# yuhogun0908/MISOnet

Measured on AMD Instinct MI355X. Metric: utterances/sec MISO1->MVDR->MISO3, 6-mic 16kHz 4s, higher is better.
Workload: dtype f32w; 1 GPU; BASELINE configs[3]: synthetic 6-mic 16 kHz 4 s, full MISO1x6 -> align -> MVDRx2 -> MISO3x2; batch_per_gpu=16, global_batch=16, frames=1001, freq_bins=129, parallelism=utterance-shard x1

## Files before the change

### include/misonet.h

```cpp
#ifndef MISONET_H_
#define MISONET_H_

#ifdef __cplusplus
extern "C" {
#endif

typedef struct misonet_net misonet_net;
typedef struct misonet_pipeline misonet_pipeline;
typedef void* misonet_stream;

enum {
  MISONET_OK = 0,
  MISONET_EINVAL = -1,
  MISONET_ESTATE = -2,
  MISONET_EHIP = -3,
  MISONET_ENOMEM = -4,
  MISONET_ENAN = -5
};

typedef struct {
  int in_ch;
  int out_ch;
  int en_ch[7];
  int de_ch[7];
  int n_freq;
  int tcn_norm;
} misonet_cfg;

const char* misonet_strerror(int code);
const char* misonet_last_error(void);
int misonet_version(void);

int misonet_net_create(const misonet_cfg* cfg, misonet_net** out);
int misonet_net_destroy(misonet_net* net);
int misonet_net_num_tensors(const misonet_net* net);
const char* misonet_net_tensor_name(const misonet_net* net, int i);
long long misonet_net_tensor_numel(const misonet_net* net, int i);
int misonet_net_set_tensor(misonet_net* net, const char* key, const float* host_data, long long numel);
int misonet_net_commit(misonet_net* net);

int misonet_net_set_precision(misonet_net* net, int mode);
int misonet_net_get_precision(const misonet_net* net);

long long misonet_net_workspace_bytes(const misonet_net* net, int n_samples, int n_frames);

int misonet_net_forward(misonet_net* net, int n_seg, const void* const* seg_dev, const int* seg_ch,
                        int B, int T, void* out_dev, void* ws_dev, long long ws_bytes, misonet_stream stream);
int misonet_net_check(misonet_net* net, const void* ws_dev, misonet_stream stream);

int misonet_net_keep_activations(misonet_net* net, int keep);
int misonet_net_buffer_plan(const misonet_net* net, int n_frames, int max_buffers, long long* offset_bytes,
                            long long* size_bytes, int* first_step, int* last_step);
int misonet_net_conv_plan(const misonet_net* net, int mode, int max_layers, int* kind);
int misonet_net_tap_shape(const misonet_net* net, const char* name, int* C, int* F);
int misonet_net_tap(misonet_net* net, const char* name, const void* ws_dev, int B, int T, float* dst_dev,
                    misonet_stream stream);

long long misonet_mvdr_workspace_bytes(int B, int F, int M);
int misonet_mvdr(const void* src_dev, const void* mix_dev, int B, int F, int M, int T, float epsi,
                 void* out_dev, void* ws_dev, long long ws_bytes, misonet_stream stream);
int misonet_mvdr_debug(const void* ws_dev, int B, int F, int M, void* steer_c128_dev, void* w_c128_dev,
                       misonet_stream stream);

long long misonet_pit_scratch_bytes(int B, int S, int F);
int misonet_pit_select(const void* anchor_dev, const void* cand_dev, int B, int S, int T, int F,
                       int* sel_dev, double* dist_dev, long long dist_bytes, misonet_stream stream);

long long misonet_css_scratch_bytes(int K, int S, int F);
int misonet_css_align(const void* est_dev, int K, int S, int T, int F, int hop_frames, const int* perm0_dev,
                      int* perm_dev, double* dist_dev, long long dist_bytes, misonet_stream stream);
int misonet_css_stitch(const float* y_dev, const int* perm_dev, int K, int S, int W, int hop, int first,
                       long long n_out, short* out_i16_dev, float* out_f32_dev, misonet_stream stream);

long long misonet_score_scratch_bytes(int B, int E, int R, long long n_or_F);
int misonet_score_wave(const void* est_dev, int est_is_i16, long long est_sb, long long est_ss, long long est_st,
                       const float* ref_dev, long long ref_sb, long long ref_ss, long long ref_st, int B, int E, int R,
                       long long n, const int* n_valid_dev, double* stats_dev, void* scratch_dev,
                       long long scratch_bytes, misonet_stream stream);
int misonet_score_spec(const void* est_dev, long long est_sb, long long est_ss, long long est_st, const void* ref_dev,
                       long long ref_sb, long long ref_ss, long long ref_st, int B, int E, int R, int T, int F,
                       double* pair_dev, int* perm_dev, double* upit_dev, void* scratch_dev, long long scratch_bytes,
                       misonet_stream stream);

long long misonet_bss_scratch_bytes(int B, int E, int R, long long n, int Q);
int misonet_bss_corr(const void* est_dev, int est_is_i16, long long est_sb, long long est_ss, long long est_st,
                     const float* ref_dev, long long ref_sb, long long ref_ss, long long ref_st, int B, int E, int R,
                     long long n, const int* n_valid_dev, int Q, double* Rrr_dev, double* Rre_dev, double* Eee_dev,
                     void* scratch_dev, long long scratch_bytes, misonet_stream stream);
int misonet_bss_solve(const double* Rrr_dev, const double* Rre_dev, const double* Eee_dev, int B, int E, int R, int Q,
                      double* T_dev, double* A_dev, int* info_dev, void* scratch_dev, long long scratch_bytes,
                      misonet_stream stream);

int misonet_pipeline_create(misonet_net* miso1, misonet_net* miso3, int num_mic, int num_spk, int ref_ch,
                            float epsi, misonet_pipeline** out);
int misonet_pipeline_destroy(misonet_pipeline* p);
long long misonet_pipeline_workspace_bytes(const misonet_pipeline* p, int B, int T);
int misonet_pipeline_run(misonet_pipeline* p, const void* mix_dev, const void* clean_dev, int B, int T,
                         void* out_dev, void* bf_dev, void* miso1_dev, void* ws_dev, long long ws_bytes,
                         misonet_stream stream);
int misonet_pipeline_check(misonet_pipeline* p, const void* ws_dev, misonet_stream stream);
int misonet_pipeline_run_wav(misonet_pipeline* p, const float* wav_dev, const float* clean_wav_dev, int B,
                             int n_samples, void* out_dev, void* bf_dev, void* miso1_dev, void* ws_dev,
                             long long ws_bytes, misonet_stream stream);

int misonet_stft_frames(int n_samples);
long long misonet_stft_workspace_bytes(int B, int M, int n_samples);
int misonet_frontend_init(void);
int misonet_stft(const float* wav_dev, int B, int n_samples, int M, void* out_dev, void* ws_dev, long long ws_bytes,
                 misonet_stream stream);

int misonet_istft(const void* spec_dev, int N, int T, void* out_i16_dev, float* out_f32_dev, misonet_stream stream);

int misonet_profile_begin(int max_launches);
int misonet_profile_end(double* ms_by_kind , long long* launches_by_kind );

int misonet_event_create(void** ev);
int misonet_event_record(void* ev, misonet_stream stream);
int misonet_event_elapsed_ms(void* start, void* stop, float* ms);
int misonet_event_destroy(void* ev);

#ifdef __cplusplus
}
#endif
#endif
```

### misonet_amd/_lib.py

```python
from __future__ import annotations

import ctypes as C
import os

_HERE = os.path.dirname(os.path.abspath(__file__))
LIB_PATH = os.environ.get("MISONET_LIB_PATH") or os.path.join(_HERE, "libmisonet_hip.so")

OK, EINVAL, ESTATE, EHIP, ENOMEM, ENAN = 0, -1, -2, -3, -4, -5


class MisonetError(RuntimeError):
    def __init__(self, code, detail):
        super().__init__(f"libmisonet_hip error {code}: {detail}")
        self.code = code


class Cfg(C.Structure):
    _fields_ = [("in_ch", C.c_int), ("out_ch", C.c_int), ("en_ch", C.c_int * 7), ("de_ch", C.c_int * 7),
                ("n_freq", C.c_int), ("tcn_norm", C.c_int)]


SIGNATURES = {
    "misonet_strerror": (C.c_char_p, [C.c_int]),
    "misonet_last_error": (C.c_char_p, []),
    "misonet_version": (C.c_int, []),
    "misonet_net_create": (C.c_int, [C.POINTER(Cfg), C.POINTER(C.c_void_p)]),
    "misonet_net_destroy": (C.c_int, [C.c_void_p]),
    "misonet_net_num_tensors": (C.c_int, [C.c_void_p]),
    "misonet_net_tensor_name": (C.c_char_p, [C.c_void_p, C.c_int]),
    "misonet_net_tensor_numel": (C.c_longlong, [C.c_void_p, C.c_int]),
    "misonet_net_set_tensor": (C.c_int, [C.c_void_p, C.c_char_p, C.c_void_p, C.c_longlong]),
    "misonet_net_commit": (C.c_int, [C.c_void_p]),
    "misonet_net_set_precision": (C.c_int, [C.c_void_p, C.c_int]),
    "misonet_net_get_precision": (C.c_int, [C.c_void_p]),
    "misonet_net_keep_activations": (C.c_int, [C.c_void_p, C.c_int]),
    "misonet_net_buffer_plan": (C.c_int, [C.c_void_p, C.c_int, C.c_int, C.POINTER(C.c_longlong), C.POINTER(C.c_longlong),
                                          C.POINTER(C.c_int), C.POINTER(C.c_int)]),
    "misonet_net_conv_plan": (C.c_int, [C.c_void_p, C.c_int, C.c_int, C.POINTER(C.c_int)]),
    "misonet_net_workspace_bytes": (C.c_longlong, [C.c_void_p, C.c_int, C.c_int]),
    "misonet_net_forward": (C.c_int, [C.c_void_p, C.c_int, C.POINTER(C.c_void_p), C.POINTER(C.c_int), C.c_int, C.c_int,
                                      C.c_void_p, C.c_void_p, C.c_longlong, C.c_void_p]),
    "misonet_net_check": (C.c_int, [C.c_void_p, C.c_void_p, C.c_void_p]),
    "misonet_net_tap_shape": (C.c_int, [C.c_void_p, C.c_char_p, C.POINTER(C.c_int), C.POINTER(C.c_int)]),
    "misonet_net_tap": (C.c_int, [C.c_void_p, C.c_char_p, C.c_void_p, C.c_int, C.c_int, C.c_void_p, C.c_void_p]),
    "misonet_mvdr_workspace_bytes": (C.c_longlong, [C.c_int, C.c_int, C.c_int]),
    "misonet_mvdr": (C.c_int, [C.c_void_p, C.c_void_p, C.c_int, C.c_int, C.c_int, C.c_int, C.c_float, C.c_void_p,
                               C.c_void_p, C.c_longlong, C.c_void_p]),
    "misonet_mvdr_debug": (C.c_int, [C.c_void_p, C.c_int, C.c_int, C.c_int, C.c_void_p, C.c_void_p, C.c_void_p]),
    "misonet_pit_scratch_bytes": (C.c_longlong, [C.c_int, C.c_int, C.c_int]),
    "misonet_pit_select": (C.c_int, [C.c_void_p, C.c_void_p, C.c_int, C.c_int, C.c_int, C.c_int, C.c_void_p, C.c_void_p,
                                     C.c_longlong, C.c_void_p]),
    "misonet_css_scratch_bytes": (C.c_longlong, [C.c_int, C.c_int, C.c_int]),
    "misonet_css_align": (C.c_int, [C.c_void_p, C.c_int, C.c_int, C.c_int, C.c_int, C.c_int, C.c_void_p, C.c_void_p,
                                    C.c_void_p, C.c_longlong, C.c_void_p]),
    "misonet_css_stitch": (C.c_int, [C.c_void_p, C.c_void_p, C.c_int, C.c_int, C.c_int, C.c_int, C.c_int, C.c_longlong,
                                     C.c_void_p, C.c_void_p, C.c_void_p]),
    "misonet_score_scratch_bytes": (C.c_longlong, [C.c_int, C.c_int, C.c_int, C.c_longlong]),
    "misonet_score_wave": (C.c_int, [C.c_void_p, C.c_int, C.c_longlong, C.c_longlong, C.c_longlong, C.c_void_p, C.c_longlong,
                                     C.c_longlong, C.c_longlong, C.c_int, C.c_int, C.c_int, C.c_longlong, C.c_void_p,
                                     C.c_void_p, C.c_void_p, C.c_longlong, C.c_void_p]),
    "misonet_score_spec": (C.c_int, [C.c_void_p, C.c_longlong, C.c_longlong, C.c_longlong, C.c_void_p, C.c_longlong,
                                     C.c_longlong, C.c_longlong, C.c_int, C.c_int, C.c_int, C.c_int, C.c_int, C.c_void_p,
                                     C.c_void_p, C.c_void_p, C.c_void_p, C.c_longlong, C.c_void_p]),
    "misonet_bss_scratch_bytes": (C.c_longlong, [C.c_int, C.c_int, C.c_int, C.c_longlong, C.c_int]),
    "misonet_bss_corr": (C.c_int, [C.c_void_p, C.c_int, C.c_longlong, C.c_longlong, C.c_longlong, C.c_void_p, C.c_longlong,
                                   C.c_longlong, C.c_longlong, C.c_int, C.c_int, C.c_int, C.c_longlong, C.c_void_p, C.c_int,
                                   C.c_void_p, C.c_void_p, C.c_void_p, C.c_void_p, C.c_longlong, C.c_void_p]),
    "misonet_bss_solve": (C.c_int, [C.c_void_p, C.c_void_p, C.c_void_p, C.c_int, C.c_int, C.c_int, C.c_int, C.c_void_p,
                                    C.c_void_p, C.c_void_p, C.c_void_p, C.c_longlong, C.c_void_p]),
    "misonet_pipeline_create": (C.c_int, [C.c_void_p, C.c_void_p, C.c_int, C.c_int, C.c_int, C.c_float,
                                          C.POINTER(C.c_void_p)]),
    "misonet_pipeline_destroy": (C.c_int, [C.c_void_p]),
    "misonet_pipeline_workspace_bytes": (C.c_longlong, [C.c_void_p, C.c_int, C.c_int]),
    "misonet_pipeline_run": (C.c_int, [C.c_void_p, C.c_void_p, C.c_void_p, C.c_int, C.c_int, C.c_void_p, C.c_void_p,
                                       C.c_void_p, C.c_void_p, C.c_longlong, C.c_void_p]),
    "misonet_pipeline_run_wav": (C.c_int, [C.c_void_p, C.c_void_p, C.c_void_p, C.c_int, C.c_int, C.c_void_p, C.c_void_p,
                                           C.c_void_p, C.c_void_p, C.c_longlong, C.c_void_p]),
    "misonet_stft_frames": (C.c_int, [C.c_int]),
    "misonet_stft_workspace_bytes": (C.c_longlong, [C.c_int, C.c_int, C.c_int]),
    "misonet_stft": (C.c_int, [C.c_void_p, C.c_int, C.c_int, C.c_int, C.c_void_p, C.c_void_p, C.c_longlong, C.c_void_p]),
    "misonet_frontend_init": (C.c_int, []),
    "misonet_istft": (C.c_int, [C.c_void_p, C.c_int, C.c_int, C.c_void_p, C.c_void_p, C.c_void_p]),
    "misonet_pipeline_check": (C.c_int, [C.c_void_p, C.c_void_p, C.c_void_p]),
    "misonet_profile_begin": (C.c_int, [C.c_int]),
    "misonet_profile_end": (C.c_int, [C.POINTER(C.c_double), C.POINTER(C.c_longlong)]),
    "misonet_event_create": (C.c_int, [C.POINTER(C.c_void_p)]),
    "misonet_event_record": (C.c_int, [C.c_void_p, C.c_void_p]),
    "misonet_event_elapsed_ms": (C.c_int, [C.c_void_p, C.c_void_p, C.POINTER(C.c_float)]),
    "misonet_event_destroy": (C.c_int, [C.c_void_p]),
}

_lib = None


def lib():
    global _lib
    if _lib is None:
        if not os.path.exists(LIB_PATH):
            raise ImportError(f"{LIB_PATH} is missing: build the HIP extension first (make -C misonet_amd/csrc). "
                              "misonet_amd has no CPU fallback.")
        import torch
        L = C.CDLL(LIB_PATH)
        for name, (res, args) in SIGNATURES.items():
            fn = getattr(L, name)
            fn.restype = res
            fn.argtypes = args
        _lib = L
    return _lib


def check(code):
    if code != OK:
        L = lib()
        detail = L.misonet_last_error().decode() or L.misonet_strerror(code).decode()
        if code == ENAN:
            raise FloatingPointError(f"libmisonet_hip: {detail}")
        raise MisonetError(code, detail)


def stream_ptr(device=None):
    import torch
    return C.c_void_p(torch.cuda.current_stream(device).cuda_stream)
```

### misonet_amd/csrc/conv.hip

```cpp
#include "conv_select.hpp"
#include <stdlib.h>
#include "conv_epilogue.hpp"

#include <atomic>
#include <type_traits>

namespace mn {

typedef float f32x16 __attribute__((ext_vector_type(16)));
typedef float f32x4 __attribute__((ext_vector_type(4)));
typedef unsigned int u32x4v __attribute__((ext_vector_type(4)));

int conv_cop(int Cout) { return Cout <= 32 ? 32 : 64; }
int conv_rows(int sf, int tr2) { return tr2 ? 3 : sf * (FT - 1) + 3; }
static int f32_rows(const ConvArgs& a) { return a.tr2 ? 5 : a.sf * (FT - 1) + 3; }

template <int NCO, int NR, int SF, bool TR2, int KFMASK, int NCP = CK / 2, bool ROW0 = false>
__device__ __forceinline__ void chunk_mfma(f32x16 (&acc)[NCO][4], const float* s_in, const float* s_w, int frel,
                                           int half, int l31) {
  constexpr int COP = NCO * 32;
  constexpr int NKF = ((KFMASK >> 0) & 1) + ((KFMASK >> 1) & 1) + ((KFMASK >> 2) & 1);
  constexpr int NSTEP = 3 * NKF * NCP;
  const float* wbase = s_w + half * COP + l31;
  const float* ibase[3];
#pragma unroll
  for (int kf = 0; kf < 3; ++kf) {
    const int rl = ROW0 ? 0 : (TR2 ? ((frel + kf) >> 1) : (SF * frel + kf));
    ibase[kf] = s_in + (half * NR + rl) * TW + l31 + 3;
  }
  float av[2][NCO], bv[2][4];
#define MN_LOAD(ST, BUF)                                                                        \
  {                                                                                             \
    constexpr int tap_ = (ST) / NCP, cp_ = (ST) % NCP;                                          \
    constexpr int kt_ = tap_ / NKF, ks_ = tap_ % NKF;                                           \
    constexpr int kf_ = (NKF == 3) ? ks_ : (NKF == 1 ? (KFMASK == 1 ? 0 : (KFMASK == 2 ? 1 : 2)) : (ks_ == 0 ? 0 : 2)); \
    _Pragma("unroll") for (int j = 0; j < NCO; ++j)                                             \
        av[BUF][j] = wbase[((kt_ * 3 + kf_) * CK + cp_ * 2) * COP + j * 32];                    \
    _Pragma("unroll") for (int q = 0; q < 4; ++q)                                               \
        bv[BUF][q] = ibase[kf_][cp_ * 2 * NR * TW + q * 32 + kt_];                              \
  }
  MN_LOAD(0, 0)
#pragma unroll
  for (int st = 0; st < NSTEP; ++st) {
    const int cur = st & 1;
    if (st + 1 < NSTEP) {
      const int nx = st + 1;
      const int tap_ = nx / NCP, cp_ = nx % NCP;
      const int kt_ = tap_ / NKF, ks_ = tap_ % NKF;
      const int kf_ = (NKF == 3) ? ks_ : (NKF == 1 ? (KFMASK == 1 ? 0 : (KFMASK == 2 ? 1 : 2)) : (ks_ == 0 ? 0 : 2));
#pragma unroll
      for (int j = 0; j < NCO; ++j) av[cur ^ 1][j] = wbase[((kt_ * 3 + kf_) * CK + cp_ * 2) * COP + j * 32];
#pragma unroll
      for (int q = 0; q < 4; ++q) bv[cur ^ 1][q] = ibase[kf_][cp_ * 2 * NR * TW + q * 32 + kt_];
    }
    __builtin_amdgcn_sched_barrier(0);
#pragma unroll
    for (int q = 0; q < 4; ++q)
#pragma unroll
      for (int j = 0; j < NCO; ++j)
        acc[j][q] = __builtin_amdgcn_mfma_f32_32x32x2f32(av[cur][j], bv[cur][q], acc[j][q], 0, 0, 0);
    __builtin_amdgcn_sched_barrier(0);
  }
#undef MN_LOAD
}

struct W1dRaw { float d[4]; };
__device__ __forceinline__ W1dRaw w1d_raw(const float* p) { W1dRaw r; r.d[0] = p[0]; r.d[1] = p[1]; r.d[2] = p[2]; r.d[3] = p[3]; return r; }
__device__ __forceinline__ void w1d_vr(const W1dRaw& r, float (&v)[4]) {
  v[0] = r.d[0] - r.d[2]; v[1] = r.d[1] + r.d[2]; v[2] = r.d[2] - r.d[1]; v[3] = r.d[1] - r.d[3];
}
template <int NR, int SF = 2, int NCP = CK / 2, int CP0 = 0, int NKF = 3>
__device__ __forceinline__ void chunk_w1d_s2(f32x16 (&acc)[4][2], const float* s_in, const float* s_w, int frel, int half, int l31) {
  const float* wb = s_w + half * 32 + l31;
  const float* ib0 = s_in + (half * NR + SF * frel) * TW + 2 * l31 + 3;
  constexpr int NSTEP = NKF * NCP;
  W1dRaw r0[2], r1[2];
  float u[2][4];
#define W1D_LOAD(ST, BUF)                                                                        \
  {                                                                                              \
    constexpr int kf_ = (ST) / NCP, cp_ = CP0 + (ST) % NCP;                                      \
    const float* ib_ = ib0 + kf_ * TW + cp_ * 2 * NR * TW;                                       \
    r0[BUF] = w1d_raw(ib_); r1[BUF] = w1d_raw(ib_ + 64);                                         \
    _Pragma("unroll") for (int nu = 0; nu < 4; ++nu) u[BUF][nu] = wb[((nu * 3 + kf_) * CK + cp_ * 2) * 32]; \
  }
  W1D_LOAD(0, 0)
#pragma unroll
  for (int st = 0; st < NSTEP; ++st) {
    const int cur = st & 1;
    if (st + 1 < NSTEP) {
      const int kf_ = (st + 1) / NCP, cp_ = CP0 + (st + 1) % NCP;
      const float* ib_ = ib0 + kf_ * TW + cp_ * 2 * NR * TW;
      r0[cur ^ 1] = w1d_raw(ib_); r1[cur ^ 1] = w1d_raw(ib_ + 64);
#pragma unroll
      for (int nu = 0; nu < 4; ++nu) u[cur ^ 1][nu] = wb[((nu * 3 + kf_) * CK + cp_ * 2) * 32];
    }
    __builtin_amdgcn_sched_barrier(0);
    float v0[4], v1[4];
    w1d_vr(r0[cur], v0);
    w1d_vr(r1[cur], v1);
#pragma unroll
    for (int nu = 0; nu < 4; ++nu) {
      acc[nu][0] = __builtin_amdgcn_mfma_f32_32x32x2f32(u[cur][nu], v0[nu], acc[nu][0], 0, 0, 0);
      acc[nu][1] = __builtin_amdgcn_mfma_f32_32x32x2f32(u[cur][nu], v1[nu], acc[nu][1], 0, 0, 0);
    }
    __builtin_amdgcn_sched_barrier(0);
  }
#undef W1D_LOAD
}
__device__ __forceinline__ void chunk_w1d_tr2(f32x16 (&acc)[4][2], const float* s_in, const float* s_w, int pr, int q, int half, int l31) {
  constexpr int NR = 3;
  const float* wb = s_w + half * 32 + l31;
  const float* ib = s_in + (half * NR + pr) * TW + 2 * l31 + 3 + 64 * q;
  W1dRaw ra[2], rb[2];
  float u0[2][4], u1[2][4], u2[2][4];
#define W1D_LOAD(CP, BUF)                                                                        \
  {                                                                                              \
    ra[BUF] = w1d_raw(ib + (CP) * 2 * NR * TW); rb[BUF] = w1d_raw(ib + (CP) * 2 * NR * TW + TW); \
    _Pragma("unroll") for (int nu = 0; nu < 4; ++nu) {                                           \
      u0[BUF][nu] = wb[((nu * 3 + 0) * CK + (CP) * 2) * 32];                                     \
      u1[BUF][nu] = wb[((nu * 3 + 1) * CK + (CP) * 2) * 32];                                     \
      u2[BUF][nu] = wb[((nu * 3 + 2) * CK + (CP) * 2) * 32];                                     \
    }                                                                                            \
  }
  W1D_LOAD(0, 0)
#pragma unroll
  for (int cp = 0; cp < CK / 2; ++cp) {
    const int cur = cp & 1;
    if (cp + 1 < CK / 2) W1D_LOAD(cp + 1, cur ^ 1)
    __builtin_amdgcn_sched_barrier(0);
    float va[4], vb[4];
    w1d_vr(ra[cur], va);
    w1d_vr(rb[cur], vb);
#pragma unroll
    for (int nu = 0; nu < 4; ++nu) {
      acc[nu][0] = __builtin_amdgcn_mfma_f32_32x32x2f32(u0[cur][nu], va[nu], acc[nu][0], 0, 0, 0);
      acc[nu][1] = __builtin_amdgcn_mfma_f32_32x32x2f32(u1[cur][nu], vb[nu], acc[nu][1], 0, 0, 0);
      acc[nu][0] = __builtin_amdgcn_mfma_f32_32x32x2f32(u2[cur][nu], vb[nu], acc[nu][0], 0, 0, 0);
    }
    __builtin_amdgcn_sched_barrier(0);
  }
#undef W1D_LOAD
}
template <int Q0, int NQ, bool ACT = true>
__device__ __forceinline__ void w1d_epilogue(const ConvArgs& a, f32x16 (&acc)[4][2], int n, int cg, int f, int tq, bool row_ok, int lane,
                                             float* s_red, const float2* s_bc) {
  const int half = lane >> 5, l31 = lane & 31;
  const int T = a.T, Tp = a.Tp;
  const int cbase = cg * 32;
  const unsigned P4 = (unsigned)a.Fout * (unsigned)Tp * 4u;
  const float* ob = a.out + (long long)n * a.out_bstride + (long long)a.out_c0 * a.Fout * Tp;
  const __amdgpu_buffer_rsrc_t rs = make_rsrc_e(reinterpret_cast<unsigned long long>(ob), (unsigned)a.Cout * P4);
  const bool all_t = row_ok && (tq + 64 * NQ <= T);
  float2 bc[16];
#pragma unroll
  for (int r = 0; r < 16; ++r) bc[r] = s_bc[(r & 3) + 8 * (r >> 2) + 4 * half];
  unsigned voff[NQ];
  bool ok[NQ], ok2[NQ];
#pragma unroll
  for (int q = 0; q < NQ; ++q) {
    const int te = tq + 64 * q + 2 * l31;
    ok[q] = row_ok && te < T;
    ok2[q] = ok[q] && te + 1 < T;
    voff[q] = ok[q] ? (unsigned)(f * Tp + te) * 4u + (unsigned)(4 * half) * P4 : 0x80000000u;
  }
  float s1[16], s2[16];
  auto body = [&](auto masked) {
    constexpr bool MASKED = decltype(masked)::value;
#pragma unroll
    for (int r = 0; r < 16; ++r) {
      const int kr = (r & 3) + 8 * (r >> 2);
      const unsigned coff = (unsigned)(cbase + kr) * P4;
      const float b = bc[r].x;
      const f32x2_t cr = {bc[r].y, bc[r].y};
      float a1 = 0.f, a2 = 0.f;
#pragma unroll
      for (int q = 0; q < NQ; ++q) {
        const float m0 = acc[0][Q0 + q][r], m1 = acc[1][Q0 + q][r], m2 = acc[2][Q0 + q][r], m3 = acc[3][Q0 + q][r];
        f32x2_t y = {(m0 + m1) + m2 + b, (m1 - m2) - m3 + b};
        if (ACT) y = elu_fast2(y) - cr;
        typedef unsigned int uu2 __attribute__((ext_vector_type(2)));
        __builtin_amdgcn_raw_buffer_store_b64(__builtin_bit_cast(uu2, y), rs, voff[q] + coff, 0, 0);
        if (!ACT) continue;
        const float ze = (!MASKED || ok[q]) ? y.x : 0.f, zo = (!MASKED || ok2[q]) ? y.y : 0.f;
        a1 += ze + zo;
        a2 = fmaf(ze, ze, fmaf(zo, zo, a2));
      }
      s1[r] = a1;
      s2[r] = a2;
    }
  };
  if (all_t || !ACT) body(std::false_type{}); else body(std::true_type{});
  if (!ACT) return;
  const float x1 = reduce16_halfwave(s1, lane);
  const float x2 = reduce16_halfwave(s2, lane);
  if ((lane & 16) == 0) {
    const int qq = lane & 15;
    const int co_l = (qq & 3) + 8 * (qq >> 2) + 4 * half;
    s_red[co_l * 2 + 0] = x1;
    s_red[co_l * 2 + 1] = x2;
  }
}

template <int NCO, int MODE, int OCTP = 0, bool HALFK = false, bool W1D = false>
__global__ __launch_bounds__(256, ((NCO == 1 && MODE != 2 && OCTP == 0 && !HALFK && !W1D) ? 3 : 2)) void conv3x3_mfma(const ConvArgs a) {
  static_assert(MODE != 2 || NCO == 1, "stride-2 transposed: two output rows per wave, 32-channel groups");
  static_assert(MODE != 4 || W1D, "MODE 4 exists in the W1D form only");
  static_assert(!W1D || (NCO == 1 && OCTP == 0 && (MODE == 0 || (!HALFK && (MODE == 1 || MODE == 2 || MODE == 3 || MODE == 4)))),
                "W1D: the frequency-strided layers and the first layer, 32-channel groups, planar output");
  constexpr int COP = NCO * 32;
  constexpr int NR = MODE == 0 ? 6 : (MODE == 1 ? 9 : (MODE == 2 ? (W1D ? 3 : 5) : (MODE == 4 ? 3 : 1)));
  constexpr int SF = (MODE == 1 || MODE == 4) ? 2 : 1;
  constexpr int NG = MODE == 4 ? 4 : 1;
  constexpr bool TR2 = MODE == 2;
  constexpr int FTO = (TR2 && !W1D) ? 2 * FT : FT;
  constexpr int NTAP = W1D ? 12 : 9;
  constexpr int NW4 = NTAP * CK * COP * NG / 4;
  constexpr int NWI = (NW4 + 255) / 256;
  extern __shared__ __align__(16) float smem[];
  float* s_in = smem;
  float* s_w = s_in + CK * NR * TW;
  float2* s_nrm = reinterpret_cast<float2*>(s_w + NTAP * CK * COP * NG);

  const int tid = threadIdx.x;
  const int lane = tid & 63;
  const int wave = __builtin_amdgcn_readfirstlane(tid >> 6);
  const ConvTile ct = conv_tile(a);
  if (!ct.valid) return;
  const int t0 = ct.t_tile * TT;
  const int f0 = ct.f_tile * FTO;
  const int n = ct.n;
  const int cg = ct.cg;
  const int T = a.T, Tp = a.Tp, Fin = a.Fin, Cin = a.Cin;
  const int nchunk = (Cin + CK - 1) / CK;
  const int fin0 = MODE == 3 ? 0 : (TR2 ? (f0 >> 1) - 1 : SF * f0 - a.padf);

  const float* in_n = a.in + (long long)n * a.in_bstride + (long long)a.in_c0 * Fin * Tp;
  const f32x4* w_g = reinterpret_cast<const f32x4*>((W1D ? a.w1d : a.w) + (long long)cg * NG * nchunk * (NTAP * CK * COP));

  const int sq = tid & 31, sci = tid >> 5;
  const int tg = t0 + 4 * sq;
  const int hr = tid >> 4, hci = (tid >> 1) & 7, hside = tid & 1;
  const int htg = hside ? t0 + TT : t0 - 1;
  const bool hok = (hr < NR) && htg >= 0 && htg < T && (fin0 + hr) >= 0 && (fin0 + hr) < Fin;

  f32x4 pin[NR];
  float ph = 0.f;
  f32x4 pw[NWI];

  const unsigned row_e = (unsigned)Tp;
  const unsigned plane_e = (unsigned)Fin * row_e;
  const unsigned long long pa = reinterpret_cast<unsigned long long>(in_n);
  const unsigned plo = __builtin_amdgcn_readfirstlane((unsigned)pa);
  const unsigned phi = __builtin_amdgcn_readfirstlane((unsigned)(pa >> 32));
  const __amdgpu_buffer_rsrc_t rs_in = __builtin_amdgcn_make_buffer_rsrc(
      reinterpret_cast<void*>(((unsigned long long)phi << 32) | plo), 0,
      __builtin_amdgcn_readfirstlane((int)((unsigned)Cin * plane_e * 4u)), 0x00020000);
  const unsigned tg_e = (unsigned)(tg < Tp ? tg : Tp - 4);
  const bool full_t = (t0 + TT <= T);
  unsigned hoff_b;
  {
    int fh = fin0 + (hr < NR ? hr : NR - 1);
    fh = fh < 0 ? 0 : (fh >= Fin ? Fin - 1 : fh);
    const int th = htg < 0 ? 0 : (htg >= Tp ? Tp - 1 : htg);
    hoff_b = ((unsigned)fh * row_e + (unsigned)th) * 4u;
  }
  unsigned roff_b[NR];
#pragma unroll
  for (int r = 0; r < NR; ++r) {
    int fin = fin0 + r;
    fin = fin < 0 ? 0 : (fin >= Fin ? Fin - 1 : fin);
    roff_b[r] = ((unsigned)fin * row_e + tg_e) * 4u;
  }

#define STAGE_ISSUE_S(KC, PIN, PH, PW)                                                                          \
  {                                                                                              \
    int c_ = (KC) * CK + sci;                                                                    \
    c_ = c_ < Cin ? c_ : Cin - 1;                                                                \
    const unsigned cb_ = (unsigned)c_ * plane_e * 4u;                                            \
    _Pragma("unroll") for (int r = 0; r < NR; ++r) PIN[r] = __builtin_bit_cast(                  \
        f32x4, __builtin_amdgcn_raw_buffer_load_b128(rs_in, cb_ + roff_b[r], 0, 0));             \
    int c2_ = (KC) * CK + hci;                                                                   \
    c2_ = c2_ < Cin ? c2_ : Cin - 1;                                                             \
    PH = __builtin_bit_cast(float, __builtin_amdgcn_raw_buffer_load_b32(                         \
        rs_in, (unsigned)c2_ * plane_e * 4u + hoff_b, 0, 0));                                    \
    const f32x4* wsrc_ = w_g + (unsigned)(KC) * (unsigned)NW4;                                   \
    _Pragma("unroll") for (int i = 0; i < NWI; ++i) {                                            \
      unsigned idx_ = tid + 256 * i;                                                             \
      if (NW4 % 256 != 0) idx_ = idx_ < (unsigned)NW4 ? idx_ : (unsigned)(NW4 - 1);              \
      if (NG > 1) {  \
        constexpr int per_ = NTAP * CK * COP / 4;                                                \
        PW[i] = w_g[(unsigned)((i / (per_ / 256)) * nchunk + (KC)) * (unsigned)per_ + tid + 256 * (i % (per_ / 256))]; \
      } else PW[i] = wsrc_[idx_];                                                                \
    }                                                                                            \
  }

#define STAGE_COMMIT_S(KC, PIN, PH, PW)                                                                         \
  {                                                                                              \
    const float2 m_ = s_nrm[(KC) * CK + sci];                                                    \
    _Pragma("unroll") for (int r = 0; r < NR; ++r) {                                             \
      const int fin_ = fin0 + r;                                                                 \
      f32x4 v_ = {0.f, 0.f, 0.f, 0.f};                                                           \
      if (fin_ >= 0 && fin_ < Fin) {                                                \
        v_.x = fmaf(PIN[r].x, m_.x, m_.y);                                                       \
        v_.y = fmaf(PIN[r].y, m_.x, m_.y);                                                       \
        v_.z = fmaf(PIN[r].z, m_.x, m_.y);                                                       \
        v_.w = fmaf(PIN[r].w, m_.x, m_.y);                                                       \
        if (!full_t) {                                                                           \
          v_.x = (tg + 0 < T) ? v_.x : 0.f;                                                      \
          v_.y = (tg + 1 < T) ? v_.y : 0.f;                                                      \
          v_.z = (tg + 2 < T) ? v_.z : 0.f;                                                      \
          v_.w = (tg + 3 < T) ? v_.w : 0.f;                                                      \
        }                                                                                        \
      }                                                                                          \
      *reinterpret_cast<f32x4*>(s_in + (sci * NR + r) * TW + 4 + 4 * sq) = v_;                   \
    }                                                                                            \
    if (hr < NR) {                                                                               \
      const float2 m2_ = s_nrm[(KC) * CK + hci];                                                 \
      s_in[(hci * NR + hr) * TW + (hside ? TT + 4 : 3)] = hok ? fmaf(PH, m2_.x, m2_.y) : 0.f;    \
    }                                                                                            \
    _Pragma("unroll") for (int i = 0; i < NWI; ++i) {                                            \
      const int idx_ = tid + 256 * i;                                                            \
      if (NW4 % 256 == 0 || idx_ < NW4) reinterpret_cast<f32x4*>(s_w)[idx_] = PW[i];             \
    }                                                                                            \
  }
#define STAGE_ISSUE(KC) STAGE_ISSUE_S(KC, pin, ph, pw)
#define STAGE_COMMIT(KC) STAGE_COMMIT_S(KC, pin, ph, pw)

  const int f = TR2 ? (W1D ? f0 + 2 * (wave >> 1) : f0 + 2 * wave) : (MODE == 4 ? f0 : f0 + wave);
  const bool row_ok = f < a.Fout;
  int nseg = (T - t0 + 31) >> 5;
  nseg = nseg > 4 ? 4 : nseg;

  f32x16 wacc[4][2];
  if (W1D) {
#pragma unroll
    for (int nu = 0; nu < 4; ++nu)
#pragma unroll
      for (int q = 0; q < 2; ++q)
#pragma unroll
        for (int r = 0; r < 16; ++r) wacc[nu][q][r] = 0.f;
  }
  f32x16 acc[NCO][4];
  f32x16 acc_o[NCO][4];
#pragma unroll
  for (int j = 0; j < NCO; ++j)
#pragma unroll
    for (int s = 0; s < 4; ++s)
#pragma unroll
      for (int r = 0; r < 16; ++r) { acc[j][s][r] = 0.f; if (TR2) acc_o[j][s][r] = 0.f; }

  const int half = lane >> 5, l31 = lane & 31;

  STAGE_ISSUE(0)
  float bias_v = 0.f;
  if (W1D && tid < 32 * NG) bias_v = __builtin_nontemporal_load(a.bias + cg * (32 * NG) + tid);
  for (int c = tid; c < nchunk * CK; c += 256) {
    float mean = 0.f, rstd = (c < Cin) ? 1.f : 0.f;
    if (c >= a.ident_c && c < Cin) {
      const dstat_t* st = a.in_stats + ((long long)n * a.in_sstride + a.in_c0 + c) * (2 * DS_NL);
      const double cnt = (double)Fin * (double)T;
      const double m = dstat_read(st) / cnt;
      double var = dstat_read(st + DS_NL) / cnt - m * m;
      var = var > 0.0 ? var : 0.0;
      mean = (float)m;
      rstd = (float)(1.0 / sqrt(var + (double)IN_EPS));
    }
    s_nrm[c] = make_float2(rstd, -mean * rstd);
  }
  float2* s_bc = s_nrm + nchunk * CK;
  if (W1D && tid < 32 * NG) s_bc[tid] = make_float2(bias_v, elu_fast(bias_v));

  __syncthreads();
  STAGE_COMMIT(0)
  __syncthreads();

  for (int kc = 0; kc < nchunk; ++kc) {
    const bool more = (kc + 1 < nchunk);
    if (more) STAGE_ISSUE(kc + 1)
    if (W1D) {
      if (row_ok) {
        if (TR2) chunk_w1d_tr2(wacc, s_in, s_w, wave >> 1, wave & 1, half, l31);
        else if (MODE == 4) chunk_w1d_s2<NR, SF>(wacc, s_in, s_w + wave * (NTAP * CK * COP), 0, half, l31);
        else if (MODE == 3) chunk_w1d_s2<NR, SF, CK / 2, 0, 1>(wacc, s_in, s_w + (2 - wave) * (CK * COP), 0, half, l31);
        else if (HALFK) {
          chunk_w1d_s2<NR, SF, CK / 4, 0>(wacc, s_in, s_w, f - f0, half, l31);
          if (kc != nchunk - 1) chunk_w1d_s2<NR, SF, CK / 4, CK / 4>(wacc, s_in, s_w, f - f0, half, l31);
        } else chunk_w1d_s2<NR, SF>(wacc, s_in, s_w, f - f0, half, l31);
      }
    } else if (row_ok) {
      if (TR2) {
        chunk_mfma<NCO, NR, SF, TR2, 5>(acc, s_in, s_w, f - f0, half, l31);
        chunk_mfma<NCO, NR, SF, TR2, 2>(acc_o, s_in, s_w, f - f0 + 1, half, l31);
      } else if (MODE == 3) {
        chunk_mfma<NCO, NR, SF, TR2, 1, CK / 2, true>(acc, s_in, s_w + (2 - wave) * (CK * COP), 0, half, l31);
      } else if (HALFK && kc == nchunk - 1) {
        chunk_mfma<NCO, NR, SF, TR2, 7, CK / 4>(acc, s_in, s_w, f - f0, half, l31);
      } else {
        chunk_mfma<NCO, NR, SF, TR2, 7>(acc, s_in, s_w, f - f0, half, l31);
      }
    }
    __syncthreads();
    if (more) {
      STAGE_COMMIT(kc + 1)
      __syncthreads();
    }
  }

  float* s_red = smem;
  if (W1D) {
    if (TR2) {
      const int q = wave & 1, rt = 2 * (wave >> 1);
      w1d_epilogue<0, 1>(a, wacc, n, cg, f, t0 + 64 * q, row_ok, lane, s_red + ((rt * 2 + q) * 32) * 2, s_bc);
      w1d_epilogue<1, 1>(a, wacc, n, cg, f + 1, t0 + 64 * q, f + 1 < a.Fout, lane, s_red + (((rt + 1) * 2 + q) * 32) * 2, s_bc);
    } else if (MODE == 4) {
      w1d_epilogue<0, 2>(a, wacc, n, cg * NG + wave, f, t0, row_ok, lane, s_red + wave * (32 * 2), s_bc + wave * 32);
    } else {
      if (MODE == 0 && !a.act) w1d_epilogue<0, 2, false>(a, wacc, n, cg, f, t0, row_ok, lane, s_red + wave * (32 * 2), s_bc);
      else w1d_epilogue<0, 2>(a, wacc, n, cg, f, t0, row_ok, lane, s_red + wave * (32 * 2), s_bc);
    }
    if (a.act) {
      __syncthreads();
      if (MODE == 4) {
        const int g = tid >> 6, co_l = (tid & 63) >> 1, which = tid & 1;
        const int co = (cg * NG + g) * 32 + co_l;
        if (co < a.Cout) {
          float tot = 0.f;
          if (f0 < a.Fout) tot += s_red[(g * 32 + co_l) * 2 + which];
          dstat_add(a.out_stats + (((long long)n * a.out_sstride + a.out_c0 + co) * 2 + which) * DS_NL, (double)tot);
        }
      } else if (tid < 64) {
        const int co_l = tid >> 1, which = tid & 1;
        const int co = cg * 32 + co_l;
        if (co < a.Cout) {
          float tot = 0.f;
          if (TR2) {
            for (int sl = 0; sl < 8; ++sl)
              if (f0 + (sl >> 1) < a.Fout) tot += s_red[(sl * 32 + co_l) * 2 + which];
          } else {
            for (int w = 0; w < FT; ++w)
              if (f0 + w < a.Fout) tot += s_red[(w * 32 + co_l) * 2 + which];
          }
          dstat_add(a.out_stats + (((long long)n * a.out_sstride + a.out_c0 + co) * 2 + which) * DS_NL, (double)tot);
        }
      }
    }
    return;
  }
  if (TR2) {
    conv_epilogue<NCO, 4, OCTP, true>(a, acc, n, cg, f, t0, row_ok, lane, s_red + (2 * wave) * (COP * 2));
    conv_epilogue<NCO, 4, OCTP, true>(a, acc_o, n, cg, f + 1, t0, f + 1 < a.Fout, lane, s_red + (2 * wave + 1) * (COP * 2));
  } else {
    conv_epilogue<NCO, 4, OCTP, true>(a, acc, n, cg, f, t0, row_ok, lane, s_red + wave * (COP * 2));
  }
  if (a.act) {
    __syncthreads();
    if (tid < COP * 2) {
      const int co_l = tid >> 1, which = tid & 1;
      const int co = cg * COP + co_l;
      if (co < a.Cout) {
        float tot = 0.f;
        for (int w = 0; w < FTO; ++w)
          if (f0 + w < a.Fout) tot += s_red[(w * COP + co_l) * 2 + which];
        dstat_add(a.out_stats + (((long long)n * a.out_sstride + a.out_c0 + co) * 2 + which) * DS_NL, (double)tot);
      }
    }
  }
}

#undef STAGE_ISSUE
#undef STAGE_COMMIT
#undef STAGE_ISSUE_S
#undef STAGE_COMMIT_S

static size_t conv_lds_bytes(int NR, int cop, int Cin, int ntap = 9) {
  const int nchunk = (Cin + CK - 1) / CK;
  return (size_t)(CK * NR * TW + ntap * CK * cop) * sizeof(float) + (size_t)(nchunk * CK + 128) * sizeof(float2);
}

template <int NCO, int MODE, int OCTP = 0, bool HALFK = false, bool W1D = false>
static hipError_t set_lds_attr() {
  return hipFuncSetAttribute(reinterpret_cast<const void*>(&conv3x3_mfma<NCO, MODE, OCTP, HALFK, W1D>),
                             hipFuncAttributeMaxDynamicSharedMemorySize, 96 * 1024);
}

hipError_t conv_init() {
  hipError_t e;
  if ((e = set_lds_attr<1, 0>()) != hipSuccess) return e;
  if ((e = set_lds_attr<1, 1>()) != hipSuccess) return e;
  if ((e = set_lds_attr<1, 2>()) != hipSuccess) return e;
  if ((e = set_lds_attr<2, 0>()) != hipSuccess) return e;
  if ((e = set_lds_attr<2, 1>()) != hipSuccess) return e;
  if ((e = set_lds_attr<1, 1, 0, false, true>()) != hipSuccess) return e;
  if ((e = set_lds_attr<1, 2, 0, false, true>()) != hipSuccess) return e;
  if ((e = set_lds_attr<1, 0, 0, true, true>()) != hipSuccess) return e;
  if ((e = set_lds_attr<1, 0, 0, false, true>()) != hipSuccess) return e;
  if ((e = set_lds_attr<1, 4, 0, false, true>()) != hipSuccess) return e;
  if ((e = set_lds_attr<1, 3, 0, false, true>()) != hipSuccess) return e;
  if ((e = set_lds_attr<1, 3>()) != hipSuccess) return e;
  if ((e = set_lds_attr<2, 3>()) != hipSuccess) return e;
  if ((e = set_lds_attr<1, 0, 3>()) != hipSuccess) return e;
  if ((e = set_lds_attr<1, 2, 3>()) != hipSuccess) return e;
  if ((e = set_lds_attr<2, 0, 3>()) != hipSuccess) return e;
#ifdef MISONET_EXPERIMENTS
  if ((e = set_lds_attr<1, 0, 4>()) != hipSuccess) return e;
  if ((e = set_lds_attr<1, 2, 4>()) != hipSuccess) return e;
  if ((e = set_lds_attr<2, 0, 4>()) != hipSuccess) return e;
  if ((e = set_lds_attr<1, 0, 4, true>()) != hipSuccess) return e;
#endif
  if ((e = set_lds_attr<1, 0, 0, true>()) != hipSuccess) return e;
  return set_lds_attr<1, 0, 3, true>();
}

int device_cus() {
  static std::atomic<int> cus[64];
  int dev = 0;
  if (hipGetDevice(&dev) != hipSuccess || dev < 0 || dev >= 64) return -1;
  int c = cus[dev].load(std::memory_order_relaxed);
  if (!c) {
    if (hipDeviceGetAttribute(&c, hipDeviceAttributeMultiprocessorCount, dev) != hipSuccess || c <= 0) return -1;
    cus[dev].store(c, std::memory_order_relaxed);
  }
  return c;
}

int conv_xcd_env() {
  static int v = -1;
  if (v < 0) v = exp_env("MISONET_XCD", 1);
  return v;
}

template <class S> static int conv_mode(const S& a) { return a.tr2 ? 2 : (a.sf == 2 ? 1 : ((a.padf == 2 && a.Fin == 1 && !a.out_oct) ? 3 : 0)); }
static bool w1d_row(const ConvShape& s) { return !s.tr2 && s.act && s.Fout == 1 && s.Fin == 3 && s.padf == 0 && s.Cout % 128 == 0; }

bool conv_w1d_ok(const ConvShape& s) {
  if (s.in_oct || s.out_oct) return false;
  if (conv_mode(s) != 0) return s.act;
  return !s.transposed && ((s.Cout <= 32 && s.Cin < 3 * CK) || w1d_row(s));
}

static int conv_xcd(int n_samples) { return (n_samples % 8 == 0) ? conv_xcd_env() : 0; }

hipError_t launch_conv_w1d(const ConvArgs& a_in, int n_samples, hipStream_t s) {
  ConvArgs a = a_in;
  const ConvShape sh = conv_shape(a);
  if (!conv_w1d_ok(sh) || !a.w1d) return hipErrorInvalidValue;
  const int mode = conv_mode(a);
  a.cop = 32;
  a.ncg = (a.Cout + 31) / 32;
  if (w1d_row(sh)) {
    a.ncg = a.Cout / 128;
    a.NR = 3;
    const dim3 grid4 = conv_grid(a, n_samples, TT, FT, conv_xcd(n_samples));
    hipLaunchKernelGGL((conv3x3_mfma<1, 4, 0, false, true>), grid4, dim3(256), conv_lds_bytes(3, 128, a.Cin, 12), s, a);
    return hipGetLastError();
  }
  a.NR = mode == 1 ? 9 : (mode == 2 ? 3 : (mode == 3 ? 1 : 6));
  const dim3 gridw = conv_grid(a, n_samples, TT, FT, conv_xcd(n_samples));
  const size_t ldsw = conv_lds_bytes(a.NR, 32, a.Cin, 12);
  const bool w1d_half = ((a.Cin - 1) % CK) < CK / 2;
  if (mode == 1) hipLaunchKernelGGL((conv3x3_mfma<1, 1, 0, false, true>), gridw, dim3(256), ldsw, s, a);
  else if (mode == 2) hipLaunchKernelGGL((conv3x3_mfma<1, 2, 0, false, true>), gridw, dim3(256), ldsw, s, a);
  else if (mode == 3) hipLaunchKernelGGL((conv3x3_mfma<1, 3, 0, false, true>), gridw, dim3(256), ldsw, s, a);
  else if (w1d_half) hipLaunchKernelGGL((conv3x3_mfma<1, 0, 0, true, true>), gridw, dim3(256), ldsw, s, a);
  else hipLaunchKernelGGL((conv3x3_mfma<1, 0, 0, false, true>), gridw, dim3(256), ldsw, s, a);
  return hipGetLastError();
}

hipError_t launch_conv(const ConvArgs& a_in, int n_samples, hipStream_t s) {
  ConvArgs a = a_in;
  if (!a.w) return hipErrorInvalidValue;
  const int mode = conv_mode(a);
  a.NR = mode == 3 ? 1 : (mode == 0 ? 6 : f32_rows(a));
  if (mode == 2 && a.cop != 32) return hipErrorInvalidValue;
  const dim3 grid = conv_grid(a, n_samples, TT, mode == 2 ? 2 * FT : FT, conv_xcd(n_samples));
  const size_t lds = conv_lds_bytes(a.NR, a.cop, a.Cin);
#define MN_LAUNCH(NCO, MODE) hipLaunchKernelGGL((conv3x3_mfma<NCO, MODE>), grid, dim3(256), lds, s, a)
#define MN_LAUNCH3(NCO, MODE) hipLaunchKernelGGL((conv3x3_mfma<NCO, MODE, 3>), grid, dim3(256), lds, s, a)
#define MN_LAUNCH4(NCO, MODE) hipLaunchKernelGGL((conv3x3_mfma<NCO, MODE, 4>), grid, dim3(256), lds, s, a)
  const bool halfk = mode == 0 && a.cop == 32 && ((a.Cin - 1) % CK) < CK / 2;
#define MN_LAUNCH_H(OCTP) hipLaunchKernelGGL((conv3x3_mfma<1, 0, OCTP, true>), grid, dim3(256), lds, s, a)
  if (a.out_oct) {
    if ((a.out_oct != 3 && a.out_oct != 4) || mode == 1 || (a.Cout & 7) || (a.out_c0 & 7) || (a.out_sstride & 7)) return hipErrorInvalidValue;
    if (a.out_oct == 3) {
      if (a.cop == 32) { if (halfk) MN_LAUNCH_H(3); else if (mode == 0) MN_LAUNCH3(1, 0); else MN_LAUNCH3(1, 2); }
      else { if (mode == 0) MN_LAUNCH3(2, 0); else return hipErrorInvalidValue; }
    } else {
#ifdef MISONET_EXPERIMENTS
      if (a.cop == 32) { if (halfk) MN_LAUNCH_H(4); else if (mode == 0) MN_LAUNCH4(1, 0); else MN_LAUNCH4(1, 2); }
      else { if (mode == 0) MN_LAUNCH4(2, 0); else return hipErrorInvalidValue; }
#else
      return hipErrorInvalidValue;
#endif
    }
  } else if (a.cop == 32) {
    if (halfk) MN_LAUNCH_H(0); else if (mode == 0) MN_LAUNCH(1, 0); else if (mode == 1) MN_LAUNCH(1, 1); else if (mode == 2) MN_LAUNCH(1, 2); else MN_LAUNCH(1, 3);
  } else {
    if (mode == 0) MN_LAUNCH(2, 0); else if (mode == 1) MN_LAUNCH(2, 1); else MN_LAUNCH(2, 3);
  }
#undef MN_LAUNCH
#undef MN_LAUNCH3
#undef MN_LAUNCH4
#undef MN_LAUNCH_H
  return hipGetLastError();
}

}
```

### misonet_amd/csrc/conv_select.hpp

```cpp
#pragma once
#include "kernels.hpp"

#ifdef MISONET_EXPERIMENTS
#define MN_ALT_MODES 1
#else
#define MN_ALT_MODES 0
#endif

namespace mn {

constexpr int CONV_NMODES = 7;
inline bool conv_mode_built(int mode) {
  return mode == 0 || mode == 3 || mode == 5 || (MN_ALT_MODES && mode >= 1 && mode < CONV_NMODES);
}

enum class ConvKind : int {
  DIRECT = 0,
  W1D,
  FEW,
  WINO,
  X6_FIRST,
  X6,
  BF16,
  BF16_DMA,
  WINO6,
};
constexpr int CONV_NKIND = 9;

struct ConvShape {
  int Cin, Cout, Fin, Fout;
  int sf, padf, tr2, act;
  bool transposed;
  int ident_c;
  bool net_input;
  int in_oct, out_oct;
};
inline ConvShape conv_shape(const ConvArgs& a, bool net_input = false) {
  return {a.Cin, a.Cout, a.Fin, a.Fout, a.sf, a.padf, a.tr2, a.act, a.padf == 2, a.ident_c, net_input, a.in_oct, a.out_oct};
}

bool conv_w1d_ok(const ConvShape& s);
bool conv_few_ok(const ConvShape& s);
bool conv_wino_ok(const ConvShape& s);
bool conv_x6_first_ok(const ConvShape& s);
bool conv_wino6_ok(const ConvShape& s);

inline ConvKind conv_select(const ConvShape& s, int mode) {
  const bool planar = mode == 0 || mode == 5 || mode == 6;
  if (s.out_oct == 3 && conv_x6_first_ok(s)) return ConvKind::X6_FIRST;
  if (s.in_oct == 3) return ConvKind::X6;
#if MN_ALT_MODES
  if (s.in_oct) return ConvKind::BF16_DMA;
  if (mode == 1 || mode == 2) return ConvKind::BF16;
  if (mode == 6 && conv_wino6_ok(s)) return ConvKind::WINO6;
#endif
  if (planar && conv_few_ok(s)) return ConvKind::FEW;
  if (mode == 5 && conv_wino_ok(s)) return ConvKind::WINO;
  if (mode == 5 && conv_w1d_ok(s)) return ConvKind::W1D;
  return ConvKind::DIRECT;
}

struct ConvWeights {
  const float* W;
  int Cin, Cout;
  bool transposed;
  int cop, ncg;
};
long long conv_image_floats(ConvKind k, const ConvWeights& c);
void conv_image_pack(ConvKind k, const ConvWeights& c, float* img);
inline long long conv_wino_ww16_at(int Cin, int Cout) { return (long long)((Cout + 31) / 32) * (Cin / 8) * 16 * 8 * 32; }
float conv_f16_wscale(const float* W, long long n);

}
```

### misonet_amd/csrc/kernels.hpp

```cpp
#pragma once
#include <hip/hip_runtime.h>
#include <stdint.h>
#include <stdlib.h>
#include "det_stats.hpp"

namespace mn {

constexpr int CK = 8;
constexpr int TT = 128;
constexpr int TW = 136;
constexpr int FT = 4;
constexpr float IN_EPS = 1e-5f;
constexpr float GLN_EPS = 1e-8f;

#ifdef MISONET_EXPERIMENTS
inline int exp_env(const char* name, int dflt) { const char* e = getenv(name); return e ? atoi(e) : dflt; }
#else
constexpr int exp_env(const char*, int dflt) { return dflt; }
#endif

inline int round_up(int x, int m) { return (x + m - 1) / m * m; }
inline int frames_pitch(int T) { return round_up(T, 32); }

struct ConvArgs {
  const float* in;
  const dstat_t* in_stats;
  float* out;
  dstat_t* out_stats;
  const float* w;
  const float* bias;
  const unsigned short* w16;
  const void* ww6;
  const float* wsm;
  const float* ww16;
  const float* w1d;
  const float* ww;
  long long in_bstride;
  long long out_bstride;
  int in_sstride, out_sstride;
  int in_c0, Cin, Fin;
  int ident_c;
  int out_c0, Cout, Fout;
  int T, Tp;
  int sf;
  int padf;
  int tr2;
  int act;
  int NR;
  int ncg;
  int cop;
  int in_oct, out_oct;
  float wscale, descale;
  const void* wps;
  long long wps_nstride;
  const float* btab;
  long long btab_nstride;
  int xcd;
  int ntx, nty, nsamp;
  unsigned long long* dbg_buf;
  int dbg;
};
struct ConvTile { int t_tile, f_tile, n, cg; bool valid; };
__device__ __forceinline__ ConvTile conv_tile(const ConvArgs& a) {
  ConvTile r;
  if (a.xcd) {
    const unsigned id = blockIdx.x;
    const unsigned xcd = id & 7u, k = id >> 3;
    const unsigned per = (unsigned)(a.ntx * a.nty * a.ncg);
    const unsigned grp = k / per;
    unsigned tile = k - grp * per;
    r.n = (int)(grp * 8u + xcd);
    r.t_tile = (int)(tile % (unsigned)a.ntx);
    tile /= (unsigned)a.ntx;
    r.cg = (int)(tile % (unsigned)a.ncg);
    r.f_tile = (int)(tile / (unsigned)a.ncg);
    r.valid = r.n < a.nsamp;
  } else {
    r.t_tile = blockIdx.x; r.f_tile = blockIdx.y;
    r.n = blockIdx.z / a.ncg; r.cg = blockIdx.z - r.n * a.ncg;
    r.valid = true;
  }
  return r;
}
inline dim3 conv_grid(ConvArgs& a, int n_samples, int tt, int ft, int xcd) {
  a.ntx = (a.T + tt - 1) / tt; a.nty = (a.Fout + ft - 1) / ft; a.nsamp = n_samples; a.xcd = xcd;
  if (xcd) return dim3((unsigned)(8 * ((n_samples + 7) / 8) * a.ntx * a.nty * a.ncg), 1, 1);
  return dim3(a.ntx, a.nty, n_samples * a.ncg);
}
int conv_xcd_env();
int device_cus();
int conv_cop(int Cout);
int conv_rows(int sf, int tr2);
hipError_t launch_conv(const ConvArgs& a, int n_samples, hipStream_t s);
hipError_t launch_conv_w1d(const ConvArgs& a, int n_samples, hipStream_t s);
hipError_t conv_init();
hipError_t launch_conv_wino(const ConvArgs& a, int n_samples, hipStream_t s);
hipError_t conv_wino_init();
hipError_t launch_conv_few(const ConvArgs& a, int n_samples, hipStream_t s);
hipError_t conv_few_init();
hipError_t launch_conv_wino6(const ConvArgs& a, int n_samples, hipStream_t s);
hipError_t conv_wino6_init();
hipError_t launch_conv_bf16(const ConvArgs& a, int n_samples, hipStream_t s);
hipError_t conv_bf16_init();
hipError_t launch_conv_bf16_dma(const ConvArgs& a, int n_samples, hipStream_t s);
hipError_t launch_conv_wprep(const ConvArgs& a, const float* wf, int n_samples, hipStream_t s);
hipError_t conv_bf16_dma_init();
hipError_t launch_conv_bf16x6(const ConvArgs& a, int n_samples, hipStream_t s);
hipError_t launch_conv_wprep6(const ConvArgs& a, const float* wf6, int n_samples, hipStream_t s);
hipError_t conv_bf16x6_init();
long long conv_bf16x6_wps_bytes(int Cin, int Cout);
hipError_t launch_conv_x6_first(const ConvArgs& a, const void* wimg, int n_samples, hipStream_t s);

int tcn_part_slots(int T);
hipError_t launch_tcn_prepare(const float* raw, long long raw_bstride, int raw_c0, const dstat_t* raw_stats, int raw_sstride,
                              float* x, double2* x_part, int C, int T, int Tp, int n_samples, hipStream_t s,
                              int raw_oct3 = 0);
hipError_t launch_tcn_dw(const float* x, const double2* x_part, int x_np, const float* wdw , const float* prelu ,
                         float* d, double2* gln_part , int C, int T, int Tp, int dilation, int n_samples, hipStream_t s,
                         int norm_kind = 0, const float* nsc = nullptr, const float* nsh = nullptr, const float2* fstat = nullptr);
hipError_t launch_tcn_cln_stats(const float* x, float2* fstat, int C, int T, int Tp, int n_samples, hipStream_t s);
hipError_t launch_tcn_pw(const float* d, const double2* gln_part, const float* gamma, const float* beta,
                         const float* wpw , const float* residual ,
                         float* y, long long y_bstride, int y_c0, double2* y_part , int C, int T, int Tp,
                         int n_samples, hipStream_t s,
                         int y_oct3_cbuf = 0, int x6 = 0);

hipError_t launch_pack(const float2* src, int B, int Mseg, int T, int F, float* dst, long long dst_bstride, int Tp,
                       int c_re, int c_im, int nshift, hipStream_t s);
hipError_t launch_unpack(const float* src, long long src_bstride, int Tp, int S, int T, int F, float2* dst, int n_samples,
                         int* nan_flag, hipStream_t s);
hipError_t launch_export(const float* src, long long src_bstride, int c0, int C, int Fq, int T, int Tp,
                         const dstat_t* stats, int sstride, int ident_c, float* dst, int n_samples, hipStream_t s,
                         int oct = 0);

struct CView {
  const float* re; const float* im;
  long long sb, sf, sm; int st;
};
struct MvdrArgs {
  CView mix;
  const float* est;
  long long est_bstride;
  const int* sel;
  CView src;
  int S;
  int B, F, M, T, Tp;
  float epsi;
};
long long mvdr_ws_bytes(int B, int S, int F, int M);
struct COut { float* re; float* im; long long ob, os, ot, of; };
hipError_t launch_mvdr(const MvdrArgs& a, const COut& out, void* ws, hipStream_t s);
hipError_t launch_mvdr_debug(const void* ws, int B, int S, int F, int M, double* steer, double* w, hipStream_t s);

struct PitArgs {
  CView a, b;
  int B, F, T;
};
hipError_t launch_pit_dist_k(const PitArgs& p, int S, int K, double* part , hipStream_t s);
hipError_t launch_pit_pick(const double* part, int F, int S, int n, double* dist , int* sel , hipStream_t s);

long long score_wave_segments(long long n);
hipError_t launch_score_wave(const void* est, int est_is_i16, const long long* es, const float* ref, const long long* rs,
                             int B, int E, int R, long long n, const int* n_valid , double* part,
                             double* stats, hipStream_t s);
hipError_t launch_score_spec(const PitArgs& p, int E, int R, double* part, double* pair, int* perm, double* upit,
                             hipStream_t s);

long long bss_corr_segments(long long n);
long long bss_solve_doubles(int R, int Q);
hipError_t launch_bss_corr(const void* est, int est_is_i16, const long long* es, const float* ref, const long long* rs, int B,
                           int E, int R, long long n, const int* n_valid , int Q, double* part, double* Rrr,
                           double* Rre, double* Eee, hipStream_t s);
hipError_t launch_bss_solve(const double* Rrr, const double* Rre, int B, int E, int R, int Q, double* T, double* A, int* info,
                            double* scratch, hipStream_t s);

}
```

### misonet_amd/csrc/net.hip

```cpp
#include "conv_select.hpp"
#include "../../include/misonet.h"

#include <math.h>
#include <cmath>
#include <algorithm>
#include <stdarg.h>
#include <stdio.h>
#include <stdlib.h>
#include <string.h>
#include <atomic>
#include <mutex>
#include <string>
#include <vector>

namespace mn {
hipError_t launch_unpack_ex(const float* src, long long src_bstride, int Tp, int S, int T, int F, int c_re0, int c_im0, int mode,
                            int M, const int* sel, float2* dst, int n_out, int* nan_flag, hipStream_t s);
hipError_t launch_compose_sel(const int* shift_sel, const int* clean_sel, int B, int M, int S, int* out, hipStream_t s);
hipError_t launch_assemble3(const float* in1, long long in1_bstride, const float* out1, long long out1_bstride,
                            const int* sel, int B, int M, int S, int ref_ch, int F, int Tp, float* in3,
                            long long in3_bstride, hipStream_t s);
hipError_t launch_stft_pack(const float* wav, int B, int L, int Mw, int T, const float* twid, float* dst,
                            long long dst_bstride, int Tp, int F, int c_re, int c_im, int nshift, hipStream_t s);
hipError_t stft_init();
hipError_t launch_istft(const void* spec, int N, int T, const float* itw, short* out_i16, float* out_f32, hipStream_t s);
hipError_t istft_init();
void istft_build_twiddles(float* tw);
int istft_twiddle_count();
void stft_build_twiddles(float* tw);
int stft_twiddle_count();
hipError_t launch_css_chain(const int* perm0, int* perm, int K, int S, hipStream_t s);
hipError_t launch_css_stitch(const float* y, const int* perm, int K, int S, int W, int hop, long long base, long long n_out,
                             short* out_i16, float* out_f32, hipStream_t s);
}

using namespace mn;

static thread_local char g_err[512] = "";
static int fail(int code, const char* fmt, ...) {
  va_list ap;
  va_start(ap, fmt);
  vsnprintf(g_err, sizeof(g_err), fmt, ap);
  va_end(ap);
  return code;
}
#define HIPCHK(expr)                                                                                    \
  do {                                                                                                  \
    hipError_t e_ = (expr);                                                                             \
    if (e_ != hipSuccess) return fail(MISONET_EHIP, "%s: %s (%s:%d)", #expr, hipGetErrorString(e_), __FILE__, __LINE__); \
  } while (0)

enum { PK_CONV = 0, PK_TCN, PK_MVDR, PK_OTHER, PK_N };
struct ProfRec { int kind; hipEvent_t e0, e1; };
struct Prof {
  bool on = false;
  std::vector<hipEvent_t> pool;
  size_t used = 0;
  std::vector<ProfRec> recs;
  bool overflow = false;
};
constexpr int MAX_DEV = 64;
static Prof g_profs[MAX_DEV];
static std::atomic<int> g_prof_any{0};
static int cur_dev() {
  int d = 0;
  if (hipGetDevice(&d) != hipSuccess || d < 0 || d >= MAX_DEV) d = 0;
  return d;
}
struct ProfScope {
  hipStream_t s; int kind; hipEvent_t e0 = nullptr, e1 = nullptr; bool active = false; Prof* pr = nullptr;
  ProfScope(hipStream_t s_, int kind_) : s(s_), kind(kind_) {
    if (!g_prof_any.load(std::memory_order_relaxed)) return;
    pr = &g_profs[cur_dev()];
    if (!pr->on) return;
    if (pr->used + 2 > pr->pool.size()) { pr->overflow = true; return; }
    e0 = pr->pool[pr->used++];
    e1 = pr->pool[pr->used++];
    active = (hipEventRecord(e0, s) == hipSuccess);
  }
  ~ProfScope() {
    if (!active) return;
    if (hipEventRecord(e1, s) == hipSuccess) pr->recs.push_back({kind, e0, e1});
  }
};

static int frontend_init();

struct Tensor {
  std::string name;
  long long numel;
  std::vector<float> host;
  bool set = false;
};

enum { B_IN = 0, B_E0, B_E1, B_E2, B_E3, B_E4, B_D0, B_D1, B_D2, B_D3, B_D4, B_D5, B_D6, B_X2, B_X3, B_X4, B_X5, B_X6,
       B_OUT, B_TXA, B_TXB, B_TD, B_TP, NBUF };

struct BufSpec { int C = 0, F = 0; };

struct ConvL {
  int in_buf, in_c0, Cin, ident_c;
  int out_buf, out_c0, Cout;
  int sf, padf, tr2, act;
  bool transposed;
  int wt, bt;
  int cop, ncg;
  ConvKind kind[CONV_NMODES];
  long long img_off[CONV_NKIND];
  long long b_off = 0;
  float wscale = 1.f;
  const float* img(const float* w_dev, ConvKind k) const { return w_dev + img_off[(int)k]; }
};

struct TcnHalf {
  int dw, prelu, gamma, beta, pw; long long o_dw, o_prelu, o_gamma, o_beta, o_pw;
  int on[4] = {-1, -1, -1, -1};
  long long o_nsc = 0, o_nsh = 0;
};
struct TcnBlock { int dilation; TcnHalf h[2]; };

struct Tap { std::string name; int buf, c0, C; bool normalised; };

struct Layout {
  int N, T, Tp;
  long long data_off[NBUF];
  long long sample_stride;
  long long in_ext_off = -1;
  long long in_ext_bstride = 0;
  long long stats_off[NBUF];
  long long tcn_xs, tcn_ps, tcn_gln;
  long long stats_doubles;
  long long data_base;
  long long wps_base, wps_nstride;
  long long btab_base, btab_nstride;
  long long fstat_base;
  long long total_bytes;
};

struct misonet_net {
  misonet_cfg cfg;
  int S;
  BufSpec bufs[NBUF];
  std::vector<Tensor> tensors;
  std::vector<ConvL> enc, dec;
  std::vector<TcnBlock> tcn;
  std::vector<Tap> taps;
  float* w_dev = nullptr;
  bool committed = false;
  bool keep_taps = false;
  int precision = 3;
};

static int find_tensor(const misonet_net* n, const std::string& name) {
  for (size_t i = 0; i < n->tensors.size(); ++i)
    if (n->tensors[i].name == name) return (int)i;
  return -1;
}
static int add_tensor(misonet_net* n, const std::string& name, long long numel) {
  Tensor t;
  t.name = name;
  t.numel = numel;
  n->tensors.push_back(t);
  return (int)n->tensors.size() - 1;
}

static ConvL make_conv(misonet_net* n, const std::string& prefix, int in_buf, int in_c0, int Cin, int ident_c, int out_buf,
                       int out_c0, int Cout, int sf, int padf, bool transposed, int act) {
  ConvL L;
  L.in_buf = in_buf; L.in_c0 = in_c0; L.Cin = Cin; L.ident_c = ident_c;
  L.out_buf = out_buf; L.out_c0 = out_c0; L.Cout = Cout;
  L.transposed = transposed;
  L.act = act;
  std::fill(L.img_off, L.img_off + CONV_NKIND, -1LL);
  if (transposed) {
    L.tr2 = (sf == 2);
    L.sf = 1;
    L.padf = 2;
  } else {
    L.tr2 = 0; L.sf = sf; L.padf = padf;
  }
  L.wt = add_tensor(n, prefix + ".weight", (long long)Cin * Cout * 9);
  L.bt = add_tensor(n, prefix + ".bias", Cout);
  L.cop = L.tr2 ? 32 : conv_cop(Cout);
  L.ncg = (Cout + L.cop - 1) / L.cop;
  return L;
}

static void add_dense(misonet_net* n, std::vector<ConvL>& v, const std::string& prefix, int buf, int init_ch, int g1, int g2,
                      int ident_c, int out_buf, int out_c0) {
  for (int i = 0; i < 5; ++i) {
    const int cin = init_ch + i * g1;
    char nm[64];
    snprintf(nm, sizeof(nm), ".conv%d.0", i + 1);
    if (i < 4)
      v.push_back(make_conv(n, prefix + nm, buf, 0, cin, ident_c, buf, cin, g1, 1, 1, false, 1));
    else
      v.push_back(make_conv(n, prefix + nm, buf, 0, cin, ident_c, out_buf, out_c0, g2, 1, 1, false, 1));
  }
}

static inline int buf_oct(int precision, int b) {
  if (precision < 2 || precision >= 5) return 0;
  const bool o = (b >= B_E0 && b <= B_E4) || (b >= B_D2 && b <= B_D6) || (b >= B_X2 && b <= B_X6);
  if (precision == 3 && (b == B_D0 || b == B_D1)) return 3;
  if (precision == 4 && b == B_E0) return 3;
  return o ? (precision == 3 ? 3 : (precision == 4 ? 4 : 1)) : 0;
}
static inline int buf_oct(const misonet_net* n, int b) { return buf_oct(n->precision, b); }

static int freq_after_conv(int F, int sf) { return (F - 3) / sf + 1; }

static int build_plan(misonet_net* n) {
  const misonet_cfg& c = n->cfg;
  if (c.n_freq != 129) return fail(MISONET_EINVAL, "n_freq must be 129 (got %d): the encoder must reduce F to one bin", c.n_freq);
  if (c.tcn_norm < 0 || c.tcn_norm > 3)
    return fail(MISONET_EINVAL, "tcn_norm must be 0 (IN), 1 (gLN), 2 (cLN) or 3 (BatchNorm1d, eval) (got %d)", c.tcn_norm);
  if (c.in_ch < 2 || c.in_ch % 2 || c.out_ch < 2 || c.out_ch % 2 || c.in_ch > 64 || c.out_ch > 32)
    return fail(MISONET_EINVAL, "in_ch/out_ch must be even and small (got %d/%d)", c.in_ch, c.out_ch);
  for (int i = 0; i < 7; ++i) {
    if (c.en_ch[i] <= 0 || c.en_ch[i] % 8 || c.de_ch[i] <= 0 || c.de_ch[i] % 8)
      return fail(MISONET_EINVAL, "bottleneck channels must be positive multiples of 8");
    if (c.en_ch[6 - i] != c.de_ch[i])
      return fail(MISONET_EINVAL, "U-Net skip concat needs en_ch[6-i] == de_ch[i] (model.py:35,99)");
  }
  if (c.en_ch[6] != 128) return fail(MISONET_EINVAL, "the TCN is TemporalConvNet(2,7,128,128,128) (model.py:31): en_ch[6] must be 128");
  for (int i = 0; i < 7; ++i)
    if (c.en_ch[i] > 128) return fail(MISONET_EINVAL, "channel counts above 128 are not supported");
  n->S = c.out_ch / 2;
  const int* en = c.en_ch;
  const int* de = c.de_ch;
  int Fe[7];
  Fe[0] = freq_after_conv(c.n_freq, 1);
  for (int b = 1; b < 7; ++b) Fe[b] = freq_after_conv(Fe[b - 1], b == 6 ? 1 : 2);
  if (Fe[6] != 1) return fail(MISONET_EINVAL, "encoder does not reduce to one frequency bin");
  n->bufs[B_IN] = {c.in_ch, c.n_freq};
  for (int b = 0; b < 5; ++b) n->bufs[B_E0 + b] = {5 * en[b], Fe[b]};
  n->bufs[B_D0] = {2 * de[0], Fe[6]};
  n->bufs[B_D1] = {2 * de[1], Fe[5]};
  for (int i = 2; i < 7; ++i) {
    n->bufs[B_D0 + i] = {6 * de[i], Fe[6 - i]};
    n->bufs[B_X2 + (i - 2)] = {2 * de[i], Fe[6 - i]};
  }
  n->bufs[B_OUT] = {c.out_ch, c.n_freq};
  for (int b = B_TXA; b <= B_TP; ++b) n->bufs[b] = {128, 1};

  char nm[96];
  for (int b = 0; b < 7; ++b) {
    const int skip_buf = B_D0 + (6 - b), skip_c0 = de[6 - b];
    const int src_buf = (b == 0) ? B_IN : B_D0 + (7 - b);
    const int src_c0 = (b == 0) ? 0 : de[7 - b];
    const int cin = (b == 0) ? c.in_ch : en[b - 1];
    if (b == 0) {
      n->enc.push_back(make_conv(n, "encoders.0.0.conv2d", B_IN, 0, cin, cin, B_E0, 0, en[0], 1, 0, false, 0));
      add_dense(n, n->enc, "encoders.0.1", B_E0, en[0], en[0], en[0], en[0], skip_buf, skip_c0);
    } else if (b < 5) {
      snprintf(nm, sizeof(nm), "encoders.%d.0.net.0", b);
      n->enc.push_back(make_conv(n, nm, src_buf, src_c0, cin, 0, B_E0 + b, 0, en[b], 2, 0, false, 1));
      snprintf(nm, sizeof(nm), "encoders.%d.1", b);
      add_dense(n, n->enc, nm, B_E0 + b, en[b], en[b], en[b], 0, skip_buf, skip_c0);
    } else {
      snprintf(nm, sizeof(nm), "encoders.%d.0.net.0", b);
      n->enc.push_back(make_conv(n, nm, src_buf, src_c0, cin, 0, skip_buf, skip_c0, en[b], b == 6 ? 1 : 2, 0, false, 1));
    }
  }
  for (int i = 0; i < 7; ++i) {
    const int buf = B_D0 + i;
    const int cin = 2 * de[i];
    const int cout = (i == 6) ? c.out_ch : de[i + 1];
    const int obuf = (i == 6) ? B_OUT : B_D0 + i + 1;
    if (i >= 2) {
      snprintf(nm, sizeof(nm), "decoders.%d.0", i);
      add_dense(n, n->dec, nm, buf, cin, cin / 2, cin, 0, B_X2 + (i - 2), 0);
      snprintf(nm, sizeof(nm), i == 6 ? "decoders.%d.1.deconv2d" : "decoders.%d.1.net.0", i);
      n->dec.push_back(make_conv(n, nm, B_X2 + (i - 2), 0, cin, 0, obuf, 0, cout, i == 6 ? 1 : 2, 0, true, i == 6 ? 0 : 1));
    } else {
      snprintf(nm, sizeof(nm), "decoders.%d.0.net.0", i);
      n->dec.push_back(make_conv(n, nm, buf, 0, cin, i == 0 ? de[0] : 0, obuf, 0, cout, i == 0 ? 1 : 2, 0, true, 1));
    }
  }
  for (int r = 0; r < 2; ++r)
    for (int x = 0; x < 7; ++x) {
      TcnBlock tb;
      tb.dilation = 1 << x;
      for (int h = 0; h < 2; ++h) {
        if (c.tcn_norm) {
          snprintf(nm, sizeof(nm), "TCN.temporal_conv_net.%d.%d.net.%d", r, x, h == 0 ? 0 : 3);
          const std::string q(nm);
          if (c.tcn_norm == 3) {
            tb.h[h].on[0] = add_tensor(n, q + ".weight", 128);
            tb.h[h].on[1] = add_tensor(n, q + ".bias", 128);
            tb.h[h].on[2] = add_tensor(n, q + ".running_mean", 128);
            tb.h[h].on[3] = add_tensor(n, q + ".running_var", 128);
          } else {
            tb.h[h].on[0] = add_tensor(n, q + ".gamma", 128);
            tb.h[h].on[1] = add_tensor(n, q + ".beta", 128);
          }
        }
        snprintf(nm, sizeof(nm), "TCN.temporal_conv_net.%d.%d.net.%d.net", r, x, h == 0 ? 2 : 5);
        const std::string p(nm);
        tb.h[h].dw = add_tensor(n, p + ".0.weight", 128 * 3);
        tb.h[h].prelu = add_tensor(n, p + ".1.weight", 1);
        tb.h[h].gamma = add_tensor(n, p + ".2.gamma", 128);
        tb.h[h].beta = add_tensor(n, p + ".2.beta", 128);
        tb.h[h].pw = add_tensor(n, p + ".3.weight", 128 * 128);
      }
      n->tcn.push_back(tb);
    }
  n->taps.push_back({"enc0_conv", B_E0, 0, en[0], false});
  for (int b = 0; b < 7; ++b) {
    snprintf(nm, sizeof(nm), "enc%d", b);
    n->taps.push_back({nm, B_D0 + (6 - b), de[6 - b], en[b], true});
  }
  n->taps.push_back({"tcn_out", B_D0, 0, 128, false});
  for (int i = 0; i < 6; ++i) {
    snprintf(nm, sizeof(nm), "dec%d", i);
    n->taps.push_back({nm, B_D0 + i + 1, 0, de[i + 1], true});
  }
  n->taps.push_back({"dec6", B_OUT, 0, c.out_ch, false});
  static const int x6first_env = exp_env("MISONET_X6_FIRST", 1);
  for (std::vector<ConvL>* v : {&n->enc, &n->dec})
    for (ConvL& l : *v)
      for (int mode = 0; mode < CONV_NMODES; ++mode) {
        const ConvShape sh = {l.Cin, l.Cout, n->bufs[l.in_buf].F, n->bufs[l.out_buf].F, l.sf, l.padf, l.tr2, l.act, l.transposed,
                              l.ident_c, l.in_buf == B_IN, buf_oct(mode, l.in_buf), buf_oct(mode, l.out_buf)};
        l.kind[mode] = conv_mode_built(mode) ? conv_select(sh, mode) : ConvKind::DIRECT;
        if (l.kind[mode] == ConvKind::X6_FIRST && !x6first_env) l.kind[mode] = ConvKind::DIRECT;
      }
  return MISONET_OK;
}

static long long align_up(long long x, long long a) { return (x + a - 1) / a * a; }

static inline long long buf_floats(const misonet_net* n, int Tp, int b) {
  const long long e = (long long)n->bufs[b].C * n->bufs[b].F * Tp;
  return buf_oct(n, b) == 3 ? e + e / 2 : e;
}
static inline long long bstride(const misonet_net* n, const Layout& L, int b) {
  if (b == B_IN && L.in_ext_off >= 0) return L.in_ext_bstride;
  return b >= B_TXA ? buf_floats(n, L.Tp, b) : L.sample_stride;
}

static void buf_lifetime(int b, int& t0, int& t1) {
  if (b == B_IN) { t0 = 0; t1 = 16; }
  else if (b >= B_E0 && b <= B_E4) { t0 = t1 = 1 + (b - B_E0); }
  else if (b >= B_D0 && b <= B_D6) { const int i = b - B_D0; t0 = 7 - i; t1 = 9 + i; }
  else if (b >= B_X2 && b <= B_X6) { t0 = t1 = 9 + 2 + (b - B_X2); }
  else { t0 = 15; t1 = 16; }
}

static Layout make_layout(const misonet_net* n, int N, int T, bool ext_in = false) {
  Layout L;
  L.N = N; L.T = T; L.Tp = frames_pitch(T);
  long long so = 0;
  for (int b = 0; b < NBUF; ++b) {
    L.stats_off[b] = so;
    so += (long long)N * n->bufs[b].C * 2 * DS_NL;
  }
  const long long tslots = tcn_part_slots(T);
  so = (so + 1) & ~1LL;
  L.tcn_xs = so;  so += 15LL * N * 128 * tslots * 2;
  L.tcn_ps = so;  so += 14LL * N * 128 * tslots * 2;
  L.tcn_gln = so; so += 28LL * N * 32 * 2;
  L.stats_doubles = so;
  L.data_base = align_up(256 + so * 8, 256);
  {
    struct Rect { int b, t0, t1; long long off, size; };
    std::vector<Rect> placed;
    std::vector<int> order;
    for (int b = 0; b < B_TXA; ++b)
      if (!(ext_in && b == B_IN)) order.push_back(b);
    L.data_off[B_IN] = 0;
    std::sort(order.begin(), order.end(), [&](int x, int y) {
      const long long sx = buf_floats(n, L.Tp, x), sy = buf_floats(n, L.Tp, y);
      return sx != sy ? sx > sy : x < y;
    });
    long long top = 0;
    for (int b : order) {
      Rect r;
      r.b = b;
      r.size = align_up(buf_floats(n, L.Tp, b), 64);
      buf_lifetime(b, r.t0, r.t1);
      if (n->keep_taps) { r.t0 = 0; r.t1 = 16; }
      std::vector<long long> cand(1, 0);
      for (const Rect& q : placed)
        if (q.t0 <= r.t1 && r.t0 <= q.t1) cand.push_back(q.off + q.size);
      std::sort(cand.begin(), cand.end());
      for (long long o : cand) {
        bool ok = true;
        for (const Rect& q : placed)
          if (q.t0 <= r.t1 && r.t0 <= q.t1 && o < q.off + q.size && q.off < o + r.size) { ok = false; break; }
        if (ok) { r.off = o; break; }
      }
      placed.push_back(r);
      L.data_off[b] = r.off;
      top = std::max(top, r.off + r.size);
    }
    L.sample_stride = top;
  }
  long long d = (long long)N * L.sample_stride;
  for (int b = B_TXA; b < NBUF; ++b) {
    L.data_off[b] = d;
    d += align_up((long long)N * buf_floats(n, L.Tp, b), 64);
  }
  long long wmax = 0, cmax = 0;
  auto scan = [&](const std::vector<ConvL>& v) {
    for (const ConvL& c : v) {
      const long long g = (c.Cout + 31) / 32, k = (c.Cin + 15) / 16;
      wmax = std::max(wmax, g * k * (2LL * 9 * 2 * 32 * 16));
      wmax = std::max(wmax, conv_bf16x6_wps_bytes((c.Cin + 7) / 8 * 8, c.Cout));
      cmax = std::max(cmax, g * 32);
    }
  };
  scan(n->enc); scan(n->dec);
  L.wps_base = align_up(L.data_base + d * 4, 256);
  L.wps_nstride = wmax;
  L.btab_base = align_up(L.wps_base + wmax * N, 256);
  L.btab_nstride = cmax * 9 * 4;
  L.fstat_base = align_up(L.btab_base + L.btab_nstride * 4 * N, 256);
  L.total_bytes = L.fstat_base + (n->cfg.tcn_norm == 2 ? (long long)N * L.Tp * 8 : 0);
  return L;
}

static inline float* buf_ptr(const Layout& L, void* ws, int b) {
  if (b == B_IN && L.in_ext_off >= 0) return reinterpret_cast<float*>(reinterpret_cast<char*>(ws) + L.in_ext_off);
  return reinterpret_cast<float*>(reinterpret_cast<char*>(ws) + L.data_base) + L.data_off[b];
}
static inline dstat_t* stats_base(void* ws) { return reinterpret_cast<dstat_t*>(reinterpret_cast<char*>(ws) + 256); }
static inline dstat_t* stats_ptr(const Layout& L, void* ws, int b) { return stats_base(ws) + L.stats_off[b]; }

static int run_conv(const misonet_net* n, const Layout& L, void* ws, const ConvL& c, hipStream_t s, int n0 = 0, int nb = -1) {
  const ConvKind kind = c.kind[n->precision];
  if (nb < 0) nb = L.N;
  ConvArgs a = {};
  a.in_bstride = bstride(n, L, c.in_buf);
  a.out_bstride = bstride(n, L, c.out_buf);
  a.in_sstride = n->bufs[c.in_buf].C;
  a.out_sstride = n->bufs[c.out_buf].C;
  a.in = buf_ptr(L, ws, c.in_buf) + (long long)n0 * a.in_bstride;
  a.out = buf_ptr(L, ws, c.out_buf) + (long long)n0 * a.out_bstride;
  a.in_stats = stats_ptr(L, ws, c.in_buf) + (long long)n0 * a.in_sstride * 2 * DS_NL;
  a.out_stats = stats_ptr(L, ws, c.out_buf) + (long long)n0 * a.out_sstride * 2 * DS_NL;
  a.bias = n->w_dev + c.b_off;
  a.in_c0 = c.in_c0; a.Cin = c.Cin; a.Fin = n->bufs[c.in_buf].F; a.ident_c = c.ident_c;
  a.out_c0 = c.out_c0; a.Cout = c.Cout; a.Fout = n->bufs[c.out_buf].F;
  a.T = L.T; a.Tp = L.Tp;
  a.sf = c.sf; a.padf = c.padf; a.tr2 = c.tr2; a.act = c.act;
  a.in_oct = buf_oct(n, c.in_buf);
  a.out_oct = buf_oct(n, c.out_buf);
  a.cop = kind == ConvKind::DIRECT ? c.cop : 32;
  a.ncg = (c.Cout + a.cop - 1) / a.cop;
  a.wscale = a.descale = 1.f;
  static const int sync_dbg = exp_env("MISONET_SYNC_DEBUG", 0);
  struct SyncDbg {
    hipStream_t s; const ConvArgs& a; int on;
    ~SyncDbg() {
      if (!on) return;
      fprintf(stderr, "[conv] Cin=%d Cout=%d Fin=%d Fout=%d T=%d in_oct=%d out_oct=%d mode=%d ... ", a.Cin, a.Cout, a.Fin, a.Fout,
              a.T, a.in_oct, a.out_oct, a.tr2 ? 2 : (a.sf == 2 ? 1 : 0));
      const hipError_t e = hipStreamSynchronize(s);
      fprintf(stderr, "%s\n", hipGetErrorString(e));
    }
  } sync_guard{s, a, sync_dbg};
  auto prep = [&](hipError_t (*launch_wprep)(const ConvArgs&, const float*, int, hipStream_t)) {
    a.wps = reinterpret_cast<char*>(ws) + L.wps_base + (long long)n0 * L.wps_nstride;
    a.wps_nstride = L.wps_nstride;
    a.btab = reinterpret_cast<float*>(reinterpret_cast<char*>(ws) + L.btab_base) + (long long)n0 * L.btab_nstride;
    a.btab_nstride = L.btab_nstride;
    ProfScope pw(s, PK_OTHER);
    return launch_wprep(a, c.img(n->w_dev, kind), nb, s);
  };
  hipError_t e = hipSuccess;
  switch (kind) {
    case ConvKind::DIRECT: { a.w = c.img(n->w_dev, kind); ProfScope ps(s, PK_CONV); e = launch_conv(a, nb, s); } break;
    case ConvKind::W1D: { a.w1d = c.img(n->w_dev, kind); ProfScope ps(s, PK_CONV); e = launch_conv_w1d(a, nb, s); } break;
    case ConvKind::FEW: { a.wsm = c.img(n->w_dev, kind); ProfScope ps(s, PK_CONV); e = launch_conv_few(a, nb, s); } break;
    case ConvKind::WINO: {
      a.ww = c.img(n->w_dev, kind);
      if ((c.Cout & 31) == 16) a.ww16 = a.ww + conv_wino_ww16_at(c.Cin, c.Cout);
      ProfScope ps(s, PK_CONV);
      e = launch_conv_wino(a, nb, s);
    } break;
    case ConvKind::X6_FIRST: { ProfScope ps(s, PK_CONV); e = launch_conv_x6_first(a, c.img(n->w_dev, kind), nb, s); } break;
    case ConvKind::X6:
      e = prep(launch_conv_wprep6);
      if (e == hipSuccess) { ProfScope ps(s, PK_CONV); e = launch_conv_bf16x6(a, nb, s); }
      break;
#if MN_ALT_MODES
    case ConvKind::BF16: {
      a.w16 = reinterpret_cast<const unsigned short*>(c.img(n->w_dev, kind));
      ProfScope ps(s, PK_CONV);
      e = launch_conv_bf16(a, nb, s);
    } break;
    case ConvKind::BF16_DMA:
      if (a.in_oct == 4) { a.wscale = c.wscale; a.descale = 1.f / c.wscale; }
      e = prep(launch_conv_wprep);
      if (e == hipSuccess) { ProfScope ps(s, PK_CONV); e = launch_conv_bf16_dma(a, nb, s); }
      break;
    case ConvKind::WINO6: { a.ww6 = c.img(n->w_dev, kind); ProfScope ps(s, PK_CONV); e = launch_conv_wino6(a, nb, s); } break;
#endif
    default: e = hipErrorInvalidValue; break;
  }
  if (e == hipErrorInvalidValue)
    return fail(MISONET_EINVAL, "conv kernel kind %d refuses the layer Cin=%d Cout=%d Fin=%d Fout=%d sf=%d padf=%d tr2=%d act=%d in_oct=%d out_oct=%d (mode %d)",
                (int)kind, a.Cin, a.Cout, a.Fin, a.Fout, a.sf, a.padf, a.tr2, a.act, a.in_oct, a.out_oct, n->precision);
  HIPCHK(e);
  return MISONET_OK;
}

static unsigned layout_stamp(const misonet_net* n, const Layout& L) {
  unsigned h = 2166136261u;
  auto mix = [&](unsigned long long v) { for (int i = 0; i < 8; ++i) { h ^= (unsigned)(v & 0xff); h *= 16777619u; v >>= 8; } };
  mix(n->keep_taps ? 1 : 0); mix((unsigned)n->precision); mix((unsigned)L.N); mix((unsigned)L.T); mix((unsigned long long)L.total_bytes);
  return h | 1u;
}

static int forward_planar(misonet_net* n, const Layout& L, void* ws, hipStream_t s) {
  HIPCHK(hipMemsetAsync(ws, 0, (size_t)(256 + L.tcn_xs * 8), s));
  HIPCHK(hipMemsetD32Async(reinterpret_cast<hipDeviceptr_t>(reinterpret_cast<char*>(ws) + 8), (int)layout_stamp(n, L), 1, s));
  static const int sub_env = exp_env("MISONET_SUBBATCH", 0);
  auto run_stack = [&](const std::vector<ConvL>& v) -> int {
    if (sub_env <= 0) {
      for (const ConvL& c : v) { int r = run_conv(n, L, ws, c, s); if (r) return r; }
      return MISONET_OK;
    }
    size_t i = 0;
    while (i < v.size()) {
      const int Fg = n->bufs[v[i].out_buf].F;
      size_t j = i;
      while (j < v.size() && n->bufs[v[j].out_buf].F == Fg) ++j;
      int sb = sub_env * (127 / (Fg > 0 ? Fg : 1));
      if (sb < 1) sb = 1;
      for (int n0 = 0; n0 < L.N; n0 += sb) {
        const int nb = (L.N - n0) < sb ? (L.N - n0) : sb;
        for (size_t k = i; k < j; ++k) { int r = run_conv(n, L, ws, v[k], s, n0, nb); if (r) return r; }
      }
      i = j;
    }
    return MISONET_OK;
  };
  { int r = run_stack(n->enc); if (r) return r; }
  {
    ProfScope ps_tcn(s, PK_TCN);
    const int N = L.N, T = L.T, Tp = L.Tp;
    double2* xs = reinterpret_cast<double2*>(stats_base(ws) + L.tcn_xs);
    double2* ps = reinterpret_cast<double2*>(stats_base(ws) + L.tcn_ps);
    double2* gl = reinterpret_cast<double2*>(stats_base(ws) + L.tcn_gln);
    const int tslots = tcn_part_slots(T);
    const long long per = (long long)N * 128 * tslots;
    const long long gper = (long long)N * 32;
    float* xa = buf_ptr(L, ws, B_TXA);
    float* xb = buf_ptr(L, ws, B_TXB);
    float* td = buf_ptr(L, ws, B_TD);
    float* tp = buf_ptr(L, ws, B_TP);
    const int skip_c0 = n->cfg.de_ch[0];
    HIPCHK(launch_tcn_prepare(buf_ptr(L, ws, B_D0), bstride(n, L, B_D0), skip_c0, stats_ptr(L, ws, B_D0),
                              n->bufs[B_D0].C, xa, xs, 128, T, Tp, N, s, buf_oct(n, B_D0) == 3));
    float* cur = xa;
    float* nxt = xb;
    static const int tcn_x6_env = exp_env("MISONET_TCN_X6", 1);
    const int tcn_x6 = (n->precision == 3 && tcn_x6_env) ? 1 : 0;
    for (int k = 0; k < 14; ++k) {
      const TcnBlock& tb = n->tcn[k];
      const float* W = n->w_dev;
      const int nk = n->cfg.tcn_norm;
      float2* fstat = reinterpret_cast<float2*>(reinterpret_cast<char*>(ws) + L.fstat_base);
      if (nk == 2) HIPCHK(launch_tcn_cln_stats(cur, fstat, 128, T, Tp, N, s));
      HIPCHK(launch_tcn_dw(cur, xs + k * per, k == 0 ? 1 : tslots, W + tb.h[0].o_dw, W + tb.h[0].o_prelu, td, gl + (2 * k) * gper,
                           128, T, Tp, tb.dilation, N, s, nk, W + tb.h[0].o_nsc, W + tb.h[0].o_nsh, fstat));
      HIPCHK(launch_tcn_pw(td, gl + (2 * k) * gper, W + tb.h[0].o_gamma, W + tb.h[0].o_beta, W + tb.h[0].o_pw,
                           nullptr, tp, 128LL * Tp, 0, ps + k * per, 128, T, Tp, N, s, 0, tcn_x6));
      if (nk == 2) HIPCHK(launch_tcn_cln_stats(tp, fstat, 128, T, Tp, N, s));
      HIPCHK(launch_tcn_dw(tp, ps + k * per, tslots, W + tb.h[1].o_dw, W + tb.h[1].o_prelu, td,
                           gl + (2 * k + 1) * gper, 128, T, Tp, tb.dilation, N, s, nk, W + tb.h[1].o_nsc, W + tb.h[1].o_nsh, fstat));
      const bool last = (k == 13);
      float* y = last ? buf_ptr(L, ws, B_D0) : nxt;
      HIPCHK(launch_tcn_pw(td, gl + (2 * k + 1) * gper, W + tb.h[1].o_gamma, W + tb.h[1].o_beta,
                           W + tb.h[1].o_pw, cur, y, last ? bstride(n, L, B_D0) : 128LL * Tp, 0,
                           xs + (k + 1) * per, 128, T, Tp, N, s, (last && buf_oct(n, B_D0) == 3) ? n->bufs[B_D0].C : 0, tcn_x6));
      float* t = cur; cur = nxt; nxt = t;
    }
  }
  { int r = run_stack(n->dec); if (r) return r; }
  return MISONET_OK;
}

extern "C" {

const char* misonet_strerror(int code) {
  switch (code) {
    case MISONET_OK: return "ok";
    case MISONET_EINVAL: return "invalid argument / unsupported geometry";
    case MISONET_ESTATE: return "invalid call order or missing tensor";
    case MISONET_EHIP: return "HIP runtime error";
    case MISONET_ENOMEM: return "workspace too small";
    case MISONET_ENAN: return "NaN in network output";
    default: return "unknown error";
  }
}
const char* misonet_last_error(void) { return g_err; }
int misonet_version(void) { return 490; }

int misonet_net_create(const misonet_cfg* cfg, misonet_net** out) {
  if (!cfg || !out) return fail(MISONET_EINVAL, "null argument");
  misonet_net* n = new misonet_net();
  n->cfg = *cfg;
  int r = build_plan(n);
  if (r) { delete n; return r; }
  *out = n;
  return MISONET_OK;
}

int misonet_net_destroy(misonet_net* n) {
  if (!n) return MISONET_OK;
  if (n->w_dev) (void)hipFree(n->w_dev);
  delete n;
  return MISONET_OK;
}

int misonet_net_num_tensors(const misonet_net* n) { return n ? (int)n->tensors.size() : 0; }
const char* misonet_net_tensor_name(const misonet_net* n, int i) {
  if (!n || i < 0 || i >= (int)n->tensors.size()) return nullptr;
  return n->tensors[i].name.c_str();
}
long long misonet_net_tensor_numel(const misonet_net* n, int i) {
  if (!n || i < 0 || i >= (int)n->tensors.size()) return -1;
  return n->tensors[i].numel;
}

int misonet_net_set_tensor(misonet_net* n, const char* key, const float* host, long long numel) {
  if (!n || !key || !host) return fail(MISONET_EINVAL, "null argument");
  const int i = find_tensor(n, key);
  if (i < 0) return fail(MISONET_EINVAL, "unexpected state_dict key '%s'", key);
  if (n->tensors[i].numel != numel)
    return fail(MISONET_EINVAL, "size mismatch for '%s': expected %lld elements, got %lld", key, n->tensors[i].numel, numel);
  n->tensors[i].host.assign(host, host + numel);
  n->tensors[i].set = true;
  n->committed = false;
  return MISONET_OK;
}

static std::atomic<int> g_wino_state[MAX_DEV] = {};
static std::mutex g_wino_mu;
static int wino_selftest() {
  const int d = cur_dev();
  int st = g_wino_state[d].load(std::memory_order_acquire);
  if (st) return st;
  std::lock_guard<std::mutex> lk(g_wino_mu);
  st = g_wino_state[d].load(std::memory_order_acquire);
  if (st) return st;
  const int Cin = 40, Cout = 48, F = 11, T = 70, Tp = frames_pitch(T), N = 2;
  std::vector<float> W((size_t)Cout * Cin * 9), bias(Cout), x((size_t)N * Cin * F * Tp);
  unsigned rng = 12345u;
  auto rnd = [&rng]() { rng = rng * 1664525u + 1013904223u; return (float)((int)(rng >> 9) - (1 << 22)) * (1.f / (1 << 22)); };
  for (float& v : W) v = 0.1f * rnd();
  for (float& v : bias) v = 0.3f * rnd();
  for (float& v : x) v = rnd();
  const ConvWeights cw = {W.data(), Cin, Cout, false, 64, 1};
  std::vector<float> wd((size_t)conv_image_floats(ConvKind::DIRECT, cw)), ww((size_t)conv_image_floats(ConvKind::WINO, cw));
  conv_image_pack(ConvKind::DIRECT, cw, wd.data());
  conv_image_pack(ConvKind::WINO, cw, ww.data());
  const size_t out_n = (size_t)N * Cout * F * Tp, st_n = (size_t)N * Cout * 2 * DS_NL;
  float *dx = nullptr, *dwd = nullptr, *dww = nullptr, *db = nullptr, *dy = nullptr;
  dstat_t* dst = nullptr;
  auto release = [&]() { (void)hipFree(dx); (void)hipFree(dwd); (void)hipFree(dww); (void)hipFree(db); (void)hipFree(dy); (void)hipFree(dst); };
  bool ok = hipMalloc(reinterpret_cast<void**>(&dx), x.size() * 4) == hipSuccess && hipMalloc(reinterpret_cast<void**>(&dwd), wd.size() * 4) == hipSuccess &&
            hipMalloc(reinterpret_cast<void**>(&dww), ww.size() * 4) == hipSuccess &&
            hipMalloc(reinterpret_cast<void**>(&db), 128 * 4) == hipSuccess &&
            hipMalloc(reinterpret_cast<void**>(&dy), 2 * out_n * 4) == hipSuccess && hipMalloc(reinterpret_cast<void**>(&dst), 2 * st_n * 8) == hipSuccess;
  std::vector<float> y(2 * out_n);
  std::vector<dstat_t> sv(2 * st_n);
  if (ok) {
    std::vector<float> b128(128, 0.f);
    std::copy(bias.begin(), bias.end(), b128.begin());
    ok = hipMemcpy(dx, x.data(), x.size() * 4, hipMemcpyHostToDevice) == hipSuccess &&
         hipMemcpy(dwd, wd.data(), wd.size() * 4, hipMemcpyHostToDevice) == hipSuccess &&
         hipMemcpy(dww, ww.data(), ww.size() * 4, hipMemcpyHostToDevice) == hipSuccess &&
         hipMemcpy(db, b128.data(), 128 * 4, hipMemcpyHostToDevice) == hipSuccess &&
         hipMemset(dy, 0, 2 * out_n * 4) == hipSuccess && hipMemset(dst, 0, 2 * st_n * 8) == hipSuccess;
  }
  if (ok) {
    ConvArgs a = {};
    a.in = dx; a.in_stats = nullptr; a.w = dwd; a.bias = db; a.ww = dww; a.ww16 = dww + conv_wino_ww16_at(Cin, Cout);
    a.in_bstride = (long long)Cin * F * Tp; a.out_bstride = (long long)Cout * F * Tp;
    a.in_sstride = Cin; a.out_sstride = Cout;
    a.in_c0 = 0; a.Cin = Cin; a.Fin = F; a.ident_c = Cin;
    a.out_c0 = 0; a.Cout = Cout; a.Fout = F; a.T = T; a.Tp = Tp;
    a.sf = 1; a.padf = 1; a.tr2 = 0; a.act = 1; a.ncg = 1; a.cop = 64;
    a.wscale = a.descale = 1.f;
    a.out = dy; a.out_stats = dst;
    ok = launch_conv_wino(a, N, nullptr) == hipSuccess;
    a.ww = nullptr; a.ww16 = nullptr; a.out = dy + out_n; a.out_stats = dst + st_n;
    ok = ok && launch_conv(a, N, nullptr) == hipSuccess && hipDeviceSynchronize() == hipSuccess &&
         hipMemcpy(y.data(), dy, 2 * out_n * 4, hipMemcpyDeviceToHost) == hipSuccess &&
         hipMemcpy(sv.data(), dst, 2 * st_n * 8, hipMemcpyDeviceToHost) == hipSuccess;
  }
  release();
  if (ok) {
    double worst = 0.0, scale = 0.0;
    for (int nn = 0; nn < N; ++nn)
      for (int c = 0; c < Cout; ++c)
        for (int f = 0; f < F; ++f)
          for (int t = 0; t < T; ++t) {
            const size_t i = (((size_t)nn * Cout + c) * F + f) * Tp + t;
            worst = std::max(worst, (double)fabsf(y[i] - y[out_n + i]));
            scale = std::max(scale, (double)fabsf(y[out_n + i]));
          }
    ok = std::isfinite(worst) && scale > 0.0 && worst <= 2e-5 * scale;
    for (size_t i = 0; ok && i < st_n / DS_NL; ++i) {
      auto rd = [](const dstat_t* p) { long long L[DS_NL]; for (int k = 0; k < DS_NL; ++k) L[k] = (long long)p[k]; return dstat_combine(L); };
      const double a1 = rd(sv.data() + i * DS_NL), a2 = rd(sv.data() + st_n + i * DS_NL);
      ok = std::isfinite(a1) && fabs(a1 - a2) <= 1e-4 * (fabs(a2) + 1.0);
    }
    if (!ok) fprintf(stderr, "[misonet] conv3x3_wino_f32 self-check FAILED on device %d (max |diff| %.3e of %.3e): mode f32w disabled\n", d, worst, scale);
  }
  st = ok ? 1 : 2;
  g_wino_state[d].store(st, std::memory_order_release);
  return st;
}

int misonet_net_commit(misonet_net* n) {
  if (!n) return fail(MISONET_EINVAL, "null argument");
  for (const Tensor& t : n->tensors)
    if (!t.set) return fail(MISONET_ESTATE, "missing state_dict key '%s'", t.name.c_str());
  long long off = 0;
  auto take = [&off](long long nfl) { long long o = off; off += (nfl + 63) / 64 * 64; return o; };
  auto conv_weights = [n](const ConvL& c) { return ConvWeights{n->tensors[c.wt].host.data(), c.Cin, c.Cout, c.transposed, c.cop, c.ncg}; };
  for (std::vector<ConvL>* v : {&n->enc, &n->dec})
    for (ConvL& c : *v) {
      std::fill(c.img_off, c.img_off + CONV_NKIND, -1LL);
      c.img_off[(int)ConvKind::DIRECT] = take(conv_image_floats(ConvKind::DIRECT, conv_weights(c)));
      c.b_off = take((long long)c.ncg * c.cop);
      for (int mode = 0; mode < CONV_NMODES; ++mode) {
        long long& o = c.img_off[(int)c.kind[mode]];
        if (conv_mode_built(mode) && o < 0) o = take(conv_image_floats(c.kind[mode], conv_weights(c)));
      }
    }
  for (TcnBlock& tb : n->tcn)
    for (int h = 0; h < 2; ++h) {
      tb.h[h].o_dw = take(128 * 3);
      tb.h[h].o_prelu = take(1);
      tb.h[h].o_gamma = take(128);
      tb.h[h].o_beta = take(128);
      tb.h[h].o_pw = take(128 * 128);
      tb.h[h].o_nsc = take(128);
      tb.h[h].o_nsh = take(128);
    }
  std::vector<float> arena((size_t)off, 0.f);
  for (std::vector<ConvL>* v : {&n->enc, &n->dec})
    for (ConvL& c : *v) {
      for (int k = 0; k < CONV_NKIND; ++k)
        if (c.img_off[k] >= 0) conv_image_pack((ConvKind)k, conv_weights(c), arena.data() + c.img_off[k]);
      const std::vector<float>& Bv = n->tensors[c.bt].host;
      for (int co = 0; co < c.ncg * c.cop; ++co) arena[c.b_off + co] = co < c.Cout ? Bv[co] : 0.f;
      if (MN_ALT_MODES) c.wscale = conv_f16_wscale(n->tensors[c.wt].host.data(), n->tensors[c.wt].numel);
    }
  for (const TcnBlock& tb : n->tcn)
    for (int h = 0; h < 2; ++h) {
      const TcnHalf& H = tb.h[h];
      memcpy(arena.data() + H.o_dw, n->tensors[H.dw].host.data(), 128 * 3 * sizeof(float));
      arena[H.o_prelu] = n->tensors[H.prelu].host[0];
      memcpy(arena.data() + H.o_gamma, n->tensors[H.gamma].host.data(), 128 * sizeof(float));
      memcpy(arena.data() + H.o_beta, n->tensors[H.beta].host.data(), 128 * sizeof(float));
      if (n->cfg.tcn_norm == 3) {
        const float *w = n->tensors[H.on[0]].host.data(), *b = n->tensors[H.on[1]].host.data(),
                    *rm = n->tensors[H.on[2]].host.data(), *rv = n->tensors[H.on[3]].host.data();
        for (int ch = 0; ch < 128; ++ch) {
          const float sc = w[ch] / sqrtf(rv[ch] + 1e-5f);
          arena[H.o_nsc + ch] = sc;
          arena[H.o_nsh + ch] = b[ch] - rm[ch] * sc;
        }
      } else if (n->cfg.tcn_norm) {
        memcpy(arena.data() + H.o_nsc, n->tensors[H.on[0]].host.data(), 128 * sizeof(float));
        memcpy(arena.data() + H.o_nsh, n->tensors[H.on[1]].host.data(), 128 * sizeof(float));
      }
      const std::vector<float>& P = n->tensors[H.pw].host;
      for (int co = 0; co < 128; ++co)
        for (int ci = 0; ci < 128; ++ci) arena[H.o_pw + (long long)ci * 128 + co] = P[(long long)co * 128 + ci];
    }
  if (n->w_dev) { (void)hipFree(n->w_dev); n->w_dev = nullptr; }
  HIPCHK(hipMalloc(reinterpret_cast<void**>(&n->w_dev), arena.size() * sizeof(float)));
  HIPCHK(hipMemcpy(n->w_dev, arena.data(), arena.size() * sizeof(float), hipMemcpyHostToDevice));
  HIPCHK(conv_init());
  HIPCHK(conv_wino_init());
  HIPCHK(conv_few_init());
#ifdef MISONET_EXPERIMENTS
  if (!exp_env("MISONET_WINO_DBG", 0))
#endif
  if (wino_selftest() != 1 && n->precision == 5)
    return fail(MISONET_ESTATE, "the f32w kernel failed its self-check on this device (see stderr): use mode 0 (f32) or 3 (bf16x6)");
#if MN_ALT_MODES
  HIPCHK(conv_wino6_init());
  HIPCHK(conv_bf16_init());
  HIPCHK(conv_bf16_dma_init());
#endif
  HIPCHK(conv_bf16x6_init());
  { int rf = frontend_init(); if (rf) return rf; }
  n->committed = true;
  return MISONET_OK;
}

int misonet_net_set_precision(misonet_net* n, int mode) {
  if (!n) return fail(MISONET_EINVAL, "null argument");
  if (mode < 0 || mode >= CONV_NMODES || !conv_mode_built(mode))
    return fail(MISONET_EINVAL, "precision mode must be 0 (f32), 3 (bf16x6) or 5 (f32w: f32 with the dense-block convs in Winograd form)%s",
                MN_ALT_MODES ? "; experiment build: also 1 / 2 (bf16x3), 4 (f16x3), 6 (bf16x6w)"
                             : "; modes 1, 2, 4, 6 exist only in the experiment build (make exp)");
  if (mode == 5 && g_wino_state[cur_dev()].load(std::memory_order_acquire) == 2)
    return fail(MISONET_ESTATE, "the f32w kernel failed its self-check on this device: mode 5 is disabled (use 0 or 3)");
  n->precision = mode;
  return MISONET_OK;
}
int misonet_net_get_precision(const misonet_net* n) { return n ? n->precision : -1; }

int misonet_net_buffer_plan(const misonet_net* n, int n_frames, int max_buffers, long long* offset_bytes,
                            long long* size_bytes, int* first_step, int* last_step) {
  if (!n || n_frames <= 0 || !offset_bytes || !size_bytes || !first_step || !last_step) return fail(MISONET_EINVAL, "null argument");
  const Layout L = make_layout(n, 1, n_frames);
  int k = 0;
  for (int b = 0; b < B_TXA && k < max_buffers; ++b, ++k) {
    offset_bytes[k] = L.data_off[b] * 4;
    size_bytes[k] = buf_floats(n, L.Tp, b) * 4;
    buf_lifetime(b, first_step[k], last_step[k]);
    if (n->keep_taps) { first_step[k] = 0; last_step[k] = 16; }
  }
  return k;
}

int misonet_net_conv_plan(const misonet_net* n, int mode, int max_layers, int* kind) {
  if (!n || !kind) return fail(MISONET_EINVAL, "null argument");
  if (mode < 0 || mode >= CONV_NMODES || !conv_mode_built(mode)) return fail(MISONET_EINVAL, "precision mode %d is not in this build", mode);
  int k = 0;
  for (const std::vector<ConvL>* v : {&n->enc, &n->dec})
    for (const ConvL& c : *v)
      if (k < max_layers) kind[k++] = (int)c.kind[mode];
  return k;
}

int misonet_net_keep_activations(misonet_net* n, int keep) {
  if (!n) return fail(MISONET_EINVAL, "null argument");
  n->keep_taps = keep != 0;
  return MISONET_OK;
}

long long misonet_net_workspace_bytes(const misonet_net* n, int n_samples, int n_frames) {
  if (!n || n_samples <= 0 || n_frames <= 0) return -1;
  return make_layout(n, n_samples, n_frames).total_bytes;
}

int misonet_net_forward(misonet_net* n, int n_seg, const void* const* seg_dev, const int* seg_ch, int B, int T,
                        void* out_dev, void* ws, long long ws_bytes, misonet_stream stream) {
  if (!n || !seg_dev || !seg_ch || !out_dev || !ws) return fail(MISONET_EINVAL, "null argument");
  if (!n->committed) return fail(MISONET_ESTATE, "misonet_net_commit has not been called");
  if (B <= 0 || T <= 0) return fail(MISONET_EINVAL, "B and T must be positive");
  int tot = 0;
  for (int i = 0; i < n_seg; ++i) tot += seg_ch[i];
  if (2 * tot != n->cfg.in_ch) return fail(MISONET_EINVAL, "input segments give %d complex channels, network expects %d", tot, n->cfg.in_ch / 2);
  const Layout L = make_layout(n, B, T);
  if (ws_bytes < L.total_bytes) return fail(MISONET_ENOMEM, "workspace %lld < %lld bytes", ws_bytes, L.total_bytes);
  hipStream_t s = reinterpret_cast<hipStream_t>(stream);
  int c0 = 0;
  for (int i = 0; i < n_seg; ++i) {
    HIPCHK(launch_pack(reinterpret_cast<const float2*>(seg_dev[i]), B, seg_ch[i], T, n->cfg.n_freq, buf_ptr(L, ws, B_IN),
                       bstride(n, L, B_IN), L.Tp, c0, tot + c0, 1, s));
    c0 += seg_ch[i];
  }
  int r = forward_planar(n, L, ws, s);
  if (r) return r;
  HIPCHK(launch_unpack(buf_ptr(L, ws, B_OUT), bstride(n, L, B_OUT), L.Tp, n->S, T, n->cfg.n_freq,
                       reinterpret_cast<float2*>(out_dev), B, reinterpret_cast<int*>(ws), s));
  return MISONET_OK;
}

int misonet_net_check(misonet_net* n, const void* ws, misonet_stream stream) {
  if (!n || !ws) return fail(MISONET_EINVAL, "null argument");
  int flag = 0;
  HIPCHK(hipMemcpyAsync(&flag, ws, sizeof(int), hipMemcpyDeviceToHost, reinterpret_cast<hipStream_t>(stream)));
  HIPCHK(hipStreamSynchronize(reinterpret_cast<hipStream_t>(stream)));
  if (flag) return fail(MISONET_ENAN, "NaN in network output");
  return MISONET_OK;
}

int misonet_net_tap_shape(const misonet_net* n, const char* name, int* C, int* F) {
  if (!n || !name) return fail(MISONET_EINVAL, "null argument");
  for (const Tap& t : n->taps)
    if (t.name == name) {
      if (C) *C = t.C;
      if (F) *F = n->bufs[t.buf].F;
      return MISONET_OK;
    }
  return fail(MISONET_EINVAL, "unknown tap '%s'", name);
}

int misonet_net_tap(misonet_net* n, const char* name, const void* ws, int B, int T, float* dst, misonet_stream stream) {
  if (!n || !name || !ws || !dst) return fail(MISONET_EINVAL, "null argument");
  const Layout L = make_layout(n, B, T);
  for (const Tap& t : n->taps)
    if (t.name == name) {
      if (!n->keep_taps && t.buf != B_OUT)
        return fail(MISONET_ESTATE, "tap '%s': activation buffers share memory; call misonet_net_keep_activations(net, 1) "
                                    "before the forward", name);
      {
        unsigned stamp = 0;
        hipStream_t s_ = reinterpret_cast<hipStream_t>(stream);
        HIPCHK(hipMemcpyAsync(&stamp, reinterpret_cast<const char*>(ws) + 8, sizeof(stamp), hipMemcpyDeviceToHost, s_));
        HIPCHK(hipStreamSynchronize(s_));
        if (stamp != layout_stamp(n, L))
          return fail(MISONET_ESTATE, "tap '%s': the forward in this workspace ran with another buffer plan / mode / shape "
                                      "(keep_activations, precision, B or T changed since); run the forward again", name);
      }
      void* w = const_cast<void*>(ws);
      HIPCHK(launch_export(buf_ptr(L, w, t.buf), bstride(n, L, t.buf), t.c0, t.C, n->bufs[t.buf].F, T, L.Tp,
                           t.normalised ? stats_ptr(L, w, t.buf) : nullptr, n->bufs[t.buf].C, 0, dst, B,
                           reinterpret_cast<hipStream_t>(stream), buf_oct(n, t.buf) >= 3 ? buf_oct(n, t.buf) : (buf_oct(n, t.buf) ? 2 : 0)));
      return MISONET_OK;
    }
  return fail(MISONET_EINVAL, "unknown tap '%s'", name);
}

long long misonet_mvdr_workspace_bytes(int B, int F, int M) { return mvdr_ws_bytes(B, 1, F, M); }

int misonet_mvdr(const void* src, const void* mix, int B, int F, int M, int T, float epsi, void* out, void* ws,
                 long long ws_bytes, misonet_stream stream) {
  if (!src || !mix || !out || !ws) return fail(MISONET_EINVAL, "null argument");
  if (M < 2 || M > 8) return fail(MISONET_EINVAL, "M must be in [2, 8] (got %d)", M);
  if (B <= 0 || F <= 0 || T <= 0) return fail(MISONET_EINVAL, "B, F, T must be positive");
  if (ws_bytes < mvdr_ws_bytes(B, 1, F, M)) return fail(MISONET_ENOMEM, "workspace too small");
  MvdrArgs a;
  const float* y = reinterpret_cast<const float*>(mix);
  const float* x = reinterpret_cast<const float*>(src);
  a.mix = {y, y + 1, 2LL * F * M * T, 2LL * M * T, 2LL * T, 2};
  a.src = {x, x + 1, 2LL * F * M * T, 2LL * M * T, 2LL * T, 2};
  a.est = nullptr; a.est_bstride = 0; a.sel = nullptr;
  a.S = 1; a.B = B; a.F = F; a.M = M; a.T = T; a.Tp = T; a.epsi = epsi;
  float* o = reinterpret_cast<float*>(out);
  COut co = {o, o + 1, 2LL * T * F, 0, 2LL * F, 2};
  HIPCHK(launch_mvdr(a, co, ws, reinterpret_cast<hipStream_t>(stream)));
  return MISONET_OK;
}

int misonet_mvdr_debug(const void* ws, int B, int F, int M, void* steer, void* w, misonet_stream stream) {
  if (!ws) return fail(MISONET_EINVAL, "null argument");
  HIPCHK(launch_mvdr_debug(ws, B, 1, F, M, reinterpret_cast<double*>(steer), reinterpret_cast<double*>(w),
                           reinterpret_cast<hipStream_t>(stream)));
  return MISONET_OK;
}

long long misonet_pit_scratch_bytes(int B, int S, int F) {
  if (B <= 0 || S <= 0 || F <= 0) return -1;
  return (long long)B * S * S * (F + 1) * (long long)sizeof(double);
}

int misonet_pit_select(const void* anchor, const void* cand, int B, int S, int T, int F, int* sel, double* dist,
                       long long dist_bytes, misonet_stream stream) {
  if (!anchor || !cand || !sel || !dist) return fail(MISONET_EINVAL, "null argument (dist is required: B*S*S*(F+1) doubles)");
  if (S < 1 || S > 4) return fail(MISONET_EINVAL, "PIT alignment enumerates S! permutations: 1 <= num_spks <= 4 (got %d)", S);
  if (B <= 0 || T <= 0 || F <= 0) return fail(MISONET_EINVAL, "B, T, F must be positive");
  if (dist_bytes < misonet_pit_scratch_bytes(B, S, F))
    return fail(MISONET_ENOMEM, "dist scratch %lld < %lld bytes (B*S*S*(F+1) doubles)", dist_bytes, misonet_pit_scratch_bytes(B, S, F));
  hipStream_t s = reinterpret_cast<hipStream_t>(stream);
  const float* a = reinterpret_cast<const float*>(anchor);
  const float* c = reinterpret_cast<const float*>(cand);
  PitArgs p;
  p.a = {a, a + 1, 2LL * S * T * F, 2, 2LL * T * F, 2 * F};
  p.b = {c, c + 1, 2LL * S * T * F, 2, 2LL * T * F, 2 * F};
  p.B = B; p.F = F; p.T = T;
  double* part = dist + (long long)B * S * S;
  HIPCHK(launch_pit_dist_k(p, S, 1, part, s));
  HIPCHK(launch_pit_pick(part, F, S, B, dist, sel, s));
  return MISONET_OK;
}

long long misonet_css_scratch_bytes(int K, int S, int F) {
  if (K <= 0 || S <= 0 || F <= 0) return -1;
  return (long long)(K - 1) * S * S * (F + 1) * (long long)sizeof(double);
}

int misonet_css_align(const void* est, int K, int S, int T, int F, int hop_frames, const int* perm0, int* perm,
                      double* dist, long long dist_bytes, misonet_stream stream) {
  if (!est || !perm) return fail(MISONET_EINVAL, "null argument");
  if (S < 1 || S > 4) return fail(MISONET_EINVAL, "the alignment enumerates S! permutations: 1 <= S <= 4 (got %d)", S);
  if (F != 129) return fail(MISONET_EINVAL, "F must be 129 (got %d)", F);
  if (K < 1 || K - 1 > 65535) return fail(MISONET_EINVAL, "K must be in [1, 65536] (got %d)", K);
  if (hop_frames <= 0 || T - hop_frames < 5)
    return fail(MISONET_EINVAL, "hop_frames must be positive and leave an overlap of at least 5 frames (T %d, hop %d)", T,
                hop_frames);
  if (K > 1 && !dist) return fail(MISONET_EINVAL, "null argument (dist is required for K > 1: (K-1)*S*S*(F+1) doubles)");
  if (dist_bytes < misonet_css_scratch_bytes(K, S, F))
    return fail(MISONET_ENOMEM, "dist scratch %lld < %lld bytes ((K-1)*S*S*(F+1) doubles)", dist_bytes,
                misonet_css_scratch_bytes(K, S, F));
  hipStream_t s = reinterpret_cast<hipStream_t>(stream);
  if (K > 1) {
    const float* e = reinterpret_cast<const float*>(est);
    const long long win = 2LL * S * T * F;
    const float* a = e + 2LL * hop_frames * F;
    const float* c = e + win;
    PitArgs p;
    p.a = {a, a + 1, win, 2, 2LL * T * F, 2 * F};
    p.b = {c, c + 1, win, 2, 2LL * T * F, 2 * F};
    p.B = K - 1; p.F = F; p.T = T - hop_frames;
    double* part = dist + (long long)(K - 1) * S * S;
    HIPCHK(launch_pit_dist_k(p, S, 1, part, s));
    HIPCHK(launch_pit_pick(part, F, S, K - 1, dist, perm + S, s));
  }
  HIPCHK(launch_css_chain(perm0, perm, K, S, s));
  return MISONET_OK;
}

int misonet_css_stitch(const float* y, const int* perm, int K, int S, int W, int hop, int first, long long n_out,
                       short* out_i16, float* out_f32, misonet_stream stream) {
  if (!y || !perm || (!out_i16 && !out_f32)) return fail(MISONET_EINVAL, "null argument");
  if (S < 1 || S > 4) return fail(MISONET_EINVAL, "S must be in [1, 4] (got %d)", S);
  if (K < 1) return fail(MISONET_EINVAL, "K must be positive (got %d)", K);
  if (W <= 0 || hop <= 0 || 2LL * hop < W || hop > W - 256)
    return fail(MISONET_EINVAL, "hop %d outside [W/2, W-256] for W = %d", hop, W);
  const long long base = first ? 0 : hop;
  const long long cap = (long long)(K - 1) * hop + W - base;
  if (n_out < 0 || n_out > cap) return fail(MISONET_EINVAL, "n_out %lld outside [0, %lld]", n_out, cap);
  if (n_out == 0) return MISONET_OK;
  HIPCHK(launch_css_stitch(y, perm, K, S, W, hop, base, n_out, out_i16, out_f32, reinterpret_cast<hipStream_t>(stream)));
  return MISONET_OK;
}

long long misonet_score_scratch_bytes(int B, int E, int R, long long n_or_F) {
  if (B <= 0 || E <= 0 || R <= 0 || n_or_F <= 0) return -1;
  const long long wave = score_wave_segments(n_or_F) * (2LL * E + 2LL * R + (long long)E * R);
  const long long spec = (n_or_F < 1024 ? n_or_F : 1024) * (long long)E * R;
  return (long long)B * (wave > spec ? wave : spec) * (long long)sizeof(double);
}

static int score_ranges(int B, int E, int R) {
  if (E < 1 || E > 5) return fail(MISONET_EINVAL, "E must be in [1, 5] (got %d): up to 4 speakers and the mixture", E);
  if (R < 1 || R > 4) return fail(MISONET_EINVAL, "R must be in [1, 4] (got %d)", R);
  if (B < 1 || B > 65535) return fail(MISONET_EINVAL, "B must be in [1, 65535] (got %d)", B);
  return MISONET_OK;
}

int misonet_score_wave(const void* est, int est_is_i16, long long est_sb, long long est_ss, long long est_st,
                       const float* ref, long long ref_sb, long long ref_ss, long long ref_st, int B, int E, int R,
                       long long n, const int* n_valid, double* stats, void* scratch, long long scratch_bytes,
                       misonet_stream stream) {
  if (!est || !ref || !stats || !scratch) return fail(MISONET_EINVAL, "null argument");
  if (const int rc = score_ranges(B, E, R)) return rc;
  if (n < 1 || n > (1LL << 40)) return fail(MISONET_EINVAL, "n must be in [1, 2^40] (got %lld)", n);
  if (est_sb < 0 || est_ss < 0 || est_st < 1 || ref_sb < 0 || ref_ss < 0 || ref_st < 1)
    return fail(MISONET_EINVAL, "strides must not be negative and the sample strides must be positive");
  const long long need = misonet_score_scratch_bytes(B, E, R, n);
  if (scratch_bytes < need)
    return fail(MISONET_ENOMEM, "scratch %lld < %lld bytes (misonet_score_scratch_bytes(B, E, R, n))", scratch_bytes, need);
  const long long es[3] = {est_sb, est_ss, est_st}, rs[3] = {ref_sb, ref_ss, ref_st};
  HIPCHK(launch_score_wave(est, est_is_i16 != 0, es, ref, rs, B, E, R, n, n_valid, reinterpret_cast<double*>(scratch), stats,
                           reinterpret_cast<hipStream_t>(stream)));
  return MISONET_OK;
}

int misonet_score_spec(const void* est, long long est_sb, long long est_ss, long long est_st, const void* ref,
                       long long ref_sb, long long ref_ss, long long ref_st, int B, int E, int R, int T, int F,
                       double* pair, int* perm, double* upit, void* scratch, long long scratch_bytes,
                       misonet_stream stream) {
  if (!est || !ref || !pair || !scratch) return fail(MISONET_EINVAL, "null argument");
  if (const int rc = score_ranges(B, E, R)) return rc;
  if (T < 1) return fail(MISONET_EINVAL, "T must be positive (got %d)", T);
  if (F < 1 || F > 1024) return fail(MISONET_EINVAL, "F must be in [1, 1024] (got %d)", F);
  if ((perm || upit) && E != R)
    return fail(MISONET_EINVAL, "the permutation pick needs as many estimates as references (E %d, R %d)", E, R);
  if (est_sb < 0 || est_ss < 0 || est_st < 1 || ref_sb < 0 || ref_ss < 0 || ref_st < 1)
    return fail(MISONET_EINVAL, "strides must not be negative and the frame strides must be positive");
  const long long need = misonet_score_scratch_bytes(B, E, R, F);
  if (scratch_bytes < need)
    return fail(MISONET_ENOMEM, "scratch %lld < %lld bytes (misonet_score_scratch_bytes(B, E, R, F))", scratch_bytes, need);
  const float* a = reinterpret_cast<const float*>(est);
  const float* c = reinterpret_cast<const float*>(ref);
  PitArgs p;
  p.a = {a, a + 1, 2 * est_sb, 2, 2 * est_ss, (int)(2 * est_st)};
  p.b = {c, c + 1, 2 * ref_sb, 2, 2 * ref_ss, (int)(2 * ref_st)};
  p.B = B; p.F = F; p.T = T;
  HIPCHK(launch_score_spec(p, E, R, reinterpret_cast<double*>(scratch), pair, perm, upit,
                           reinterpret_cast<hipStream_t>(stream)));
  return MISONET_OK;
}

static int bss_ranges(int B, int E, int R, int Q) {
  if (E < 1 || E > 4) return fail(MISONET_EINVAL, "E must be in [1, 4] (got %d)", E);
  if (R < 1 || R > 4) return fail(MISONET_EINVAL, "R must be in [1, 4] (got %d)", R);
  if (B < 1 || B > 4096) return fail(MISONET_EINVAL, "B must be in [1, 4096] (got %d)", B);
  if (Q < 16 || Q > 1024 || Q % 16) return fail(MISONET_EINVAL, "Q must be a multiple of 16 in [16, 1024] (got %d)", Q);
  return MISONET_OK;
}

long long misonet_bss_scratch_bytes(int B, int E, int R, long long n, int Q) {
  if (B < 1 || B > 4096 || E < 1 || E > 4 || R < 1 || R > 4 || Q < 16 || Q > 1024 || Q % 16 || n < 1 || n > (1LL << 24)) return -1;
  const long long corr = bss_corr_segments(n) * ((long long)R * R + (long long)R * E + E) * Q;
  const long long sys = bss_solve_doubles(R, Q);
  return (long long)B * (corr > sys ? corr : sys) * (long long)sizeof(double);
}

int misonet_bss_corr(const void* est, int est_is_i16, long long est_sb, long long est_ss, long long est_st, const float* ref,
                     long long ref_sb, long long ref_ss, long long ref_st, int B, int E, int R, long long n,
                     const int* n_valid, int Q, double* Rrr, double* Rre, double* Eee, void* scratch,
                     long long scratch_bytes, misonet_stream stream) {
  if (!est || !ref || !Rrr || !Rre || !Eee || !scratch) return fail(MISONET_EINVAL, "null argument");
  if (const int rc = bss_ranges(B, E, R, Q)) return rc;
  if (n < 1 || n > (1LL << 24)) return fail(MISONET_EINVAL, "n must be in [1, 2^24] (got %lld)", n);
  if (est_sb < 0 || est_ss < 0 || est_st < 1 || ref_sb < 0 || ref_ss < 0 || ref_st < 1)
    return fail(MISONET_EINVAL, "strides must not be negative and the sample strides must be positive");
  const long long need = misonet_bss_scratch_bytes(B, E, R, n, Q);
  if (scratch_bytes < need)
    return fail(MISONET_ENOMEM, "scratch %lld < %lld bytes (misonet_bss_scratch_bytes(B, E, R, n, Q))", scratch_bytes, need);
  const long long es[3] = {est_sb, est_ss, est_st}, rs[3] = {ref_sb, ref_ss, ref_st};
  HIPCHK(launch_bss_corr(est, est_is_i16 != 0, es, ref, rs, B, E, R, n, n_valid, Q, reinterpret_cast<double*>(scratch), Rrr, Rre,
                         Eee, reinterpret_cast<hipStream_t>(stream)));
  return MISONET_OK;
}

int misonet_bss_solve(const double* Rrr, const double* Rre, const double* Eee, int B, int E, int R, int Q, double* T, double* A,
                      int* info, void* scratch, long long scratch_bytes, misonet_stream stream) {
  if (!Rrr || !Rre || !Eee || !T || !A || !info || !scratch) return fail(MISONET_EINVAL, "null argument");
  if (const int rc = bss_ranges(B, E, R, Q)) return rc;
  const long long need = misonet_bss_scratch_bytes(B, E, R, 1, Q);
  if (scratch_bytes < need)
    return fail(MISONET_ENOMEM, "scratch %lld < %lld bytes (misonet_bss_scratch_bytes(B, E, R, 1, Q))", scratch_bytes, need);
  HIPCHK(launch_bss_solve(Rrr, Rre, B, E, R, Q, T, A, info, reinterpret_cast<double*>(scratch),
                          reinterpret_cast<hipStream_t>(stream)));
  return MISONET_OK;
}

static std::atomic<float*> g_twid[MAX_DEV] = {};
static std::atomic<float*> g_itwid[MAX_DEV] = {};
static std::mutex g_front_mu;
static int frontend_init() {
  const int d = cur_dev();
  std::lock_guard<std::mutex> lk(g_front_mu);
  if (!g_twid[d].load(std::memory_order_acquire)) {
    std::vector<float> tw((size_t)stft_twiddle_count());
    stft_build_twiddles(tw.data());
    float* p = nullptr;
    HIPCHK(hipMalloc(reinterpret_cast<void**>(&p), tw.size() * sizeof(float)));
    HIPCHK(hipMemcpy(p, tw.data(), tw.size() * sizeof(float), hipMemcpyHostToDevice));
    HIPCHK(stft_init());
    g_twid[d].store(p, std::memory_order_release);
  }
  if (!g_itwid[d].load(std::memory_order_acquire)) {
    std::vector<float> tw((size_t)istft_twiddle_count());
    istft_build_twiddles(tw.data());
    float* p = nullptr;
    HIPCHK(hipMalloc(reinterpret_cast<void**>(&p), tw.size() * sizeof(float)));
    HIPCHK(hipMemcpy(p, tw.data(), tw.size() * sizeof(float), hipMemcpyHostToDevice));
    HIPCHK(istft_init());
    g_itwid[d].store(p, std::memory_order_release);
  }
  return MISONET_OK;
}
int misonet_frontend_init(void) { return frontend_init(); }

static int get_twiddles(const float** out) {
  const int d = cur_dev();
  if (!g_twid[d].load(std::memory_order_acquire)) { int r = frontend_init(); if (r) return r; }
  *out = g_twid[d].load(std::memory_order_acquire);
  return MISONET_OK;
}
static int get_itwiddles(const float** out) {
  const int d = cur_dev();
  if (!g_itwid[d].load(std::memory_order_acquire)) { int r = frontend_init(); if (r) return r; }
  *out = g_itwid[d].load(std::memory_order_acquire);
  return MISONET_OK;
}

int misonet_istft(const void* spec_dev, int N, int T, void* out_i16_dev, float* out_f32_dev, misonet_stream stream) {
  if (!spec_dev || (!out_i16_dev && !out_f32_dev)) return fail(MISONET_EINVAL, "null argument");
  if (N <= 0 || T < 2) return fail(MISONET_EINVAL, "N must be positive and T >= 2 (got %d, %d)", N, T);
  const float* tw;
  int r = get_itwiddles(&tw);
  if (r) return r;
  HIPCHK(launch_istft(spec_dev, N, T, tw, reinterpret_cast<short*>(out_i16_dev), out_f32_dev,
                      reinterpret_cast<hipStream_t>(stream)));
  return MISONET_OK;
}

int misonet_stft_frames(int n_samples) { return n_samples > 0 ? n_samples / 64 + 1 : -1; }

long long misonet_stft_workspace_bytes(int B, int M, int n_samples) {
  const int T = misonet_stft_frames(n_samples);
  if (B <= 0 || M <= 0 || T <= 0) return -1;
  return (long long)B * 2 * M * 129 * frames_pitch(T) * 4;
}

int misonet_stft(const float* wav_dev, int B, int n_samples, int M, void* out_c64, void* ws, long long ws_bytes,
                 misonet_stream stream) {
  if (!wav_dev || !out_c64 || !ws) return fail(MISONET_EINVAL, "null argument");
  if (B <= 0 || M <= 0 || M > 64 || n_samples <= 0) return fail(MISONET_EINVAL, "bad B / M / n_samples");
  if (ws_bytes < misonet_stft_workspace_bytes(B, M, n_samples)) return fail(MISONET_ENOMEM, "workspace too small");
  const int T = misonet_stft_frames(n_samples), Tp = frames_pitch(T), F = 129;
  const float* tw;
  int r = get_twiddles(&tw);
  if (r) return r;
  hipStream_t s = reinterpret_cast<hipStream_t>(stream);
  float* planar = reinterpret_cast<float*>(ws);
  const long long bs = 2LL * M * F * Tp;
  HIPCHK(launch_stft_pack(wav_dev, B, n_samples, M, T, tw, planar, bs, Tp, F, 0, M, 1, s));
  HIPCHK(launch_unpack(planar, bs, Tp, M, T, F, reinterpret_cast<float2*>(out_c64), B, nullptr, s));
  return MISONET_OK;
}

struct misonet_pipeline {
  misonet_net* n1;
  misonet_net* n3;
  int M, S, ref_ch;
  float epsi;
};

struct PipeLayout {
  Layout L1, L3;
  long long off_ws1, off_ws3, off_clean, off_dist, off_sel, off_mvdr, total;
  long long clean_bstride;
};

static PipeLayout pipe_layout(const misonet_pipeline* p, int B, int T) {
  PipeLayout P;
  P.L1 = make_layout(p->n1, B * p->M, T);
  if (p->n3) P.L3 = make_layout(p->n3, B * p->S, T, true);
  else { P.L3 = Layout(); P.L3.total_bytes = 0; }
  const int F = p->n1->cfg.n_freq, Tp = P.L1.Tp;
  long long o = 256;
  P.off_dist = o;  o += align_up((long long)(B * p->M + B) * p->S * p->S * (F + 1) * 8, 256);
  P.off_sel = o;   o += align_up((long long)(B * p->M * p->S * 2 + B * p->S) * 4, 256);
  P.off_mvdr = o;  o += align_up(mvdr_ws_bytes(B, p->S, F, p->M), 256);
  P.clean_bstride = (long long)2 * p->S * F * Tp;
  P.off_clean = o; o += align_up(P.clean_bstride * B * 4, 256);
  P.L3.in_ext_bstride = p->n3 ? (long long)p->n3->cfg.in_ch * F * Tp : 0;
  const long long in3_bytes = align_up(P.L3.in_ext_bstride * B * p->S * 4, 256);
  P.off_ws1 = o;   o += align_up(std::max(P.L1.total_bytes, P.L3.total_bytes), 256);
  P.off_ws3 = P.off_ws1;
  P.L3.in_ext_off = o - P.off_ws3;
  o += in3_bytes;
  P.total = o;
  return P;
}

int misonet_pipeline_create(misonet_net* n1, misonet_net* n3, int num_mic, int num_spk, int ref_ch, float epsi,
                            misonet_pipeline** out) {
  if (!n1 || !out) return fail(MISONET_EINVAL, "null argument");
  if (num_spk < 1 || num_spk > 4) return fail(MISONET_EINVAL, "num_spk must be in [1, 4] (PIT enumerates num_spk! permutations)");
  if (num_mic < 2 || num_mic > 8) return fail(MISONET_EINVAL, "num_mic must be in [2, 8]");
  if (ref_ch < 0 || ref_ch >= num_mic) return fail(MISONET_EINVAL, "ref_ch out of range");
  if (n1->cfg.in_ch != 2 * num_mic || n1->cfg.out_ch != 2 * num_spk)
    return fail(MISONET_EINVAL, "MISO_1 geometry does not match num_mic/num_spk");
  if (n3 && (n3->cfg.in_ch != 2 * (num_mic + 2) || n3->cfg.out_ch != 2))
    return fail(MISONET_EINVAL, "MISO_3 geometry must be in_ch = 2*(num_mic+2), out_ch = 2");
  { int rf = frontend_init(); if (rf) return rf; }
  misonet_pipeline* p = new misonet_pipeline{n1, n3, num_mic, num_spk, ref_ch, epsi};
  *out = p;
  return MISONET_OK;
}
int misonet_pipeline_destroy(misonet_pipeline* p) { delete p; return MISONET_OK; }

long long misonet_pipeline_workspace_bytes(const misonet_pipeline* p, int B, int T) {
  if (!p || B <= 0 || T <= 0) return -1;
  return pipe_layout(p, B, T).total;
}

static int pipeline_run_impl(misonet_pipeline* p, const void* mix, const void* clean, const float* wav,
                             const float* clean_wav, int n_samples, int B, int T, void* out, void* bf_out,
                             void* miso1_out, void* ws, long long ws_bytes, misonet_stream stream) {
  if (!p || (!mix && !wav) || (!out && !miso1_out) || !ws) return fail(MISONET_EINVAL, "null argument");
  if (!p->n1->committed || (p->n3 && !p->n3->committed)) return fail(MISONET_ESTATE, "networks not committed");
  if (!p->n3 && (out || bf_out))
    return fail(MISONET_ESTATE, "this pipeline was created without MISO_3 (separation only): out and bf_out must be NULL");
  if (B <= 0 || T <= 0) return fail(MISONET_EINVAL, "B and T must be positive");
  const PipeLayout P = pipe_layout(p, B, T);
  if (ws_bytes < P.total) return fail(MISONET_ENOMEM, "workspace %lld < %lld bytes", ws_bytes, P.total);
  hipStream_t s = reinterpret_cast<hipStream_t>(stream);
  char* base = reinterpret_cast<char*>(ws);
  void* ws1 = base + P.off_ws1;
  void* ws3 = base + P.off_ws3;
  const int M = p->M, S = p->S, F = p->n1->cfg.n_freq, Tp = P.L1.Tp;
  misonet_net *n1 = p->n1, *n3 = p->n3;
  double* dist_shift = reinterpret_cast<double*>(base + P.off_dist);
  double* dist_clean = dist_shift + (long long)B * M * S * S;
  double* part_shift = dist_clean + (long long)B * S * S;
  double* part_clean = part_shift + (long long)B * M * F * S * S;
  int* sel_shift = reinterpret_cast<int*>(base + P.off_sel);
  int* sel_final = sel_shift + (long long)B * M * S;
  int* sel_clean = sel_final + (long long)B * M * S;
  HIPCHK(hipMemsetAsync(base, 0, 256, s));

  float* in1 = buf_ptr(P.L1, ws1, B_IN);
  const long long in1_bs = bstride(n1, P.L1, B_IN);
  const float* tw = nullptr;
  if (wav) { int rt = get_twiddles(&tw); if (rt) return rt; }
  if (wav) HIPCHK(launch_stft_pack(wav, B, n_samples, M, T, tw, in1, in1_bs, Tp, F, 0, M, M, s));
  else HIPCHK(launch_pack(reinterpret_cast<const float2*>(mix), B, M, T, F, in1, in1_bs, Tp, 0, M, M, s));
  int r = forward_planar(n1, P.L1, ws1, s);
  if (r) return r;
  float* out1 = buf_ptr(P.L1, ws1, B_OUT);
  const long long out1_bs = bstride(n1, P.L1, B_OUT);
  const long long plane = (long long)F * Tp;

  {
    PitArgs q;
    const float* anc = out1 + (long long)p->ref_ch * out1_bs;
    q.a = {anc, anc + S * plane, (long long)M * out1_bs, Tp, plane, 1};
    q.b = {out1, out1 + S * plane, out1_bs, Tp, plane, 1};
    q.B = B; q.F = F; q.T = T;
    HIPCHK(launch_pit_dist_k(q, S, M, part_shift, s));
    HIPCHK(launch_pit_pick(part_shift, F, S, B * M, dist_shift, sel_shift, s));
  }
  if (clean || clean_wav) {
    float* cl = reinterpret_cast<float*>(base + P.off_clean);
    if (clean_wav) HIPCHK(launch_stft_pack(clean_wav, B, n_samples, S, T, tw, cl, P.clean_bstride, Tp, F, 0, S, 1, s));
    else HIPCHK(launch_pack(reinterpret_cast<const float2*>(clean), B, S, T, F, cl, P.clean_bstride, Tp, 0, S, 1, s));
    PitArgs q;
    const float* cand = out1 + (long long)p->ref_ch * out1_bs;
    q.a = {cl, cl + S * plane, P.clean_bstride, Tp, plane, 1};
    q.b = {cand, cand + S * plane, (long long)M * out1_bs, Tp, plane, 1};
    q.B = B; q.F = F; q.T = T;
    HIPCHK(launch_pit_dist_k(q, S, 1, part_clean, s));
    HIPCHK(launch_pit_pick(part_clean, F, S, B, dist_clean, sel_clean, s));
  }
  HIPCHK(launch_compose_sel(sel_shift, (clean || clean_wav) ? sel_clean : nullptr, B, M, S, sel_final, s));

  if (out) {
    float* in3 = buf_ptr(P.L3, ws3, B_IN);
    const long long in3_bs = bstride(n3, P.L3, B_IN);
    HIPCHK(launch_assemble3(in1, in1_bs, out1, out1_bs, sel_final, B, M, S, p->ref_ch, F, Tp, in3, in3_bs, s));

    {
      MvdrArgs a;
      a.mix = {in1, in1 + (long long)M * plane, (long long)M * in1_bs, Tp, plane, 1};
      a.est = out1; a.est_bstride = out1_bs; a.sel = sel_final;
      a.src = {nullptr, nullptr, 0, 0, 0, 1};
      a.S = S; a.B = B; a.F = F; a.M = M; a.T = T; a.Tp = Tp; a.epsi = p->epsi;
      COut co = {in3 + (long long)M * plane, in3 + (long long)(2 * M + 2) * plane, (long long)S * in3_bs, in3_bs, 1, Tp};
      ProfScope ps(s, PK_MVDR);
      HIPCHK(launch_mvdr(a, co, base + P.off_mvdr, s));
    }
    if (miso1_out)
      HIPCHK(launch_unpack_ex(out1, out1_bs, Tp, S, T, F, 0, S, 1, M, sel_final, reinterpret_cast<float2*>(miso1_out),
                              B * S * M, reinterpret_cast<int*>(base), s));
    r = forward_planar(n3, P.L3, ws3, s);
    if (r) return r;
    HIPCHK(launch_unpack(buf_ptr(P.L3, ws3, B_OUT), bstride(n3, P.L3, B_OUT), Tp, 1, T, F, reinterpret_cast<float2*>(out),
                         B * S, reinterpret_cast<int*>(base), s));
    if (bf_out)
      HIPCHK(launch_unpack_ex(in3, in3_bs, Tp, 1, T, F, M, 2 * M + 2, 0, 1, nullptr,
                              reinterpret_cast<float2*>(bf_out), B * S, reinterpret_cast<int*>(base), s));
  } else if (miso1_out) {
    HIPCHK(launch_unpack_ex(out1, out1_bs, Tp, S, T, F, 0, S, 1, M, sel_final, reinterpret_cast<float2*>(miso1_out),
                            B * S * M, reinterpret_cast<int*>(base), s));
  }
  return MISONET_OK;
}

int misonet_pipeline_run(misonet_pipeline* p, const void* mix, const void* clean, int B, int T, void* out, void* bf_out,
                         void* miso1_out, void* ws, long long ws_bytes, misonet_stream stream) {
  return pipeline_run_impl(p, mix, clean, nullptr, nullptr, 0, B, T, out, bf_out, miso1_out, ws, ws_bytes, stream);
}

int misonet_pipeline_run_wav(misonet_pipeline* p, const float* wav, const float* clean_wav, int B, int n_samples,
                             void* out, void* bf_out, void* miso1_out, void* ws, long long ws_bytes,
                             misonet_stream stream) {
  if (n_samples <= 0) return fail(MISONET_EINVAL, "n_samples must be positive");
  return pipeline_run_impl(p, nullptr, nullptr, wav, clean_wav, n_samples, B, misonet_stft_frames(n_samples), out, bf_out,
                           miso1_out, ws, ws_bytes, stream);
}

int misonet_pipeline_check(misonet_pipeline* p, const void* ws, misonet_stream stream) {
  if (!p || !ws) return fail(MISONET_EINVAL, "null argument");
  int flag = 0;
  HIPCHK(hipMemcpyAsync(&flag, ws, sizeof(int), hipMemcpyDeviceToHost, reinterpret_cast<hipStream_t>(stream)));
  HIPCHK(hipStreamSynchronize(reinterpret_cast<hipStream_t>(stream)));
  if (flag) return fail(MISONET_ENAN, "NaN in pipeline output");
  return MISONET_OK;
}

int misonet_profile_begin(int max_launches) {
  if (max_launches <= 0) return fail(MISONET_EINVAL, "max_launches must be positive");
  Prof& pr = g_profs[cur_dev()];
  while (pr.pool.size() < (size_t)max_launches * 2) {
    hipEvent_t e;
    HIPCHK(hipEventCreate(&e));
    pr.pool.push_back(e);
  }
  pr.used = 0;
  pr.recs.clear();
  pr.overflow = false;
  if (!pr.on) g_prof_any.fetch_add(1);
  pr.on = true;
  return MISONET_OK;
}
int misonet_profile_end(double* ms_by_kind, long long* launches_by_kind) {
  Prof& pr = g_profs[cur_dev()];
  if (pr.on) g_prof_any.fetch_sub(1);
  pr.on = false;
  if (!ms_by_kind || !launches_by_kind) return fail(MISONET_EINVAL, "null argument");
  for (int k = 0; k < PK_N; ++k) { ms_by_kind[k] = 0.0; launches_by_kind[k] = 0; }
  for (const ProfRec& r : pr.recs) {
    HIPCHK(hipEventSynchronize(r.e1));
    float ms = 0.f;
    HIPCHK(hipEventElapsedTime(&ms, r.e0, r.e1));
    ms_by_kind[r.kind] += ms;
    launches_by_kind[r.kind] += 1;
  }
  if (pr.overflow) return fail(MISONET_ENOMEM, "profile event pool exhausted");
  return MISONET_OK;
}

int misonet_event_create(void** ev) {
  hipEvent_t e;
  HIPCHK(hipEventCreate(&e));
  *ev = e;
  return MISONET_OK;
}
int misonet_event_record(void* ev, misonet_stream stream) {
  HIPCHK(hipEventRecord(reinterpret_cast<hipEvent_t>(ev), reinterpret_cast<hipStream_t>(stream)));
  return MISONET_OK;
}
int misonet_event_elapsed_ms(void* start, void* stop, float* ms) {
  HIPCHK(hipEventSynchronize(reinterpret_cast<hipEvent_t>(stop)));
  HIPCHK(hipEventElapsedTime(ms, reinterpret_cast<hipEvent_t>(start), reinterpret_cast<hipEvent_t>(stop)));
  return MISONET_OK;
}
int misonet_event_destroy(void* ev) {
  HIPCHK(hipEventDestroy(reinterpret_cast<hipEvent_t>(ev)));
  return MISONET_OK;
}

}
```

Before: 149.2 utt/s.

## Add persistent streaming kernel for strided W1D conv layers with cross-tile prefetch

Adds a persistent conv3x3_w1d_stream kernel that launches about two workgroups per CU, each walking a contiguous range of (sample, channel group, freq tile, time tile) work items. It prefetches the next tile's first input chunk while the current tile's epilogue runs, and rebuilds bias/stat tables only when a new run starts. The goal is to cut launch tail and idle time between tiles and to overlap global loads with epilogue stores. The W1D helper code moves into a shared header, and a runtime switch plus a schedule query API are exposed. The costs are extra synchronisation, LDS sized by Cin, and a fixed grid that can leave CUs unbalanced.

```diff
diff --git a/include/misonet.h b/include/misonet.h
--- a/include/misonet.h
+++ b/include/misonet.h
@@ -52,6 +52,8 @@
 int misonet_net_buffer_plan(const misonet_net* net, int n_frames, int max_buffers, long long* offset_bytes,
                             long long* size_bytes, int* first_step, int* last_step);
 int misonet_net_conv_plan(const misonet_net* net, int mode, int max_layers, int* kind);
+int misonet_strided_stream(int on);
+int misonet_strided_schedule(int ntx, int nty, int ncg, int n_samples, int grid, int wg, int max_tiles, int* tiles);
 int misonet_net_tap_shape(const misonet_net* net, const char* name, int* C, int* F);
 int misonet_net_tap(misonet_net* net, const char* name, const void* ws_dev, int B, int T, float* dst_dev,
                     misonet_stream stream);
diff --git a/misonet_amd/_lib.py b/misonet_amd/_lib.py
--- a/misonet_amd/_lib.py
+++ b/misonet_amd/_lib.py
@@ -37,6 +37,8 @@
     "misonet_net_buffer_plan": (C.c_int, [C.c_void_p, C.c_int, C.c_int, C.POINTER(C.c_longlong), C.POINTER(C.c_longlong),
                                           C.POINTER(C.c_int), C.POINTER(C.c_int)]),
     "misonet_net_conv_plan": (C.c_int, [C.c_void_p, C.c_int, C.c_int, C.POINTER(C.c_int)]),
+    "misonet_strided_stream": (C.c_int, [C.c_int]),
+    "misonet_strided_schedule": (C.c_int, [C.c_int, C.c_int, C.c_int, C.c_int, C.c_int, C.c_int, C.c_int, C.POINTER(C.c_int)]),
     "misonet_net_workspace_bytes": (C.c_longlong, [C.c_void_p, C.c_int, C.c_int]),
     "misonet_net_forward": (C.c_int, [C.c_void_p, C.c_int, C.POINTER(C.c_void_p), C.POINTER(C.c_int), C.c_int, C.c_int,
                                       C.c_void_p, C.c_void_p, C.c_longlong, C.c_void_p]),
diff --git a/misonet_amd/csrc/conv.hip b/misonet_amd/csrc/conv.hip
--- a/misonet_amd/csrc/conv.hip
+++ b/misonet_amd/csrc/conv.hip
@@ -1,15 +1,12 @@
 #include "conv_select.hpp"
 #include <stdlib.h>
 #include "conv_epilogue.hpp"
+#include "conv_w1d.hpp"
 
 #include <atomic>
 #include <type_traits>
 
 namespace mn {
-
-typedef float f32x16 __attribute__((ext_vector_type(16)));
-typedef float f32x4 __attribute__((ext_vector_type(4)));
-typedef unsigned int u32x4v __attribute__((ext_vector_type(4)));
 
 int conv_cop(int Cout) { return Cout <= 32 ? 32 : 64; }
 int conv_rows(int sf, int tr2) { return tr2 ? 3 : sf * (FT - 1) + 3; }
@@ -62,143 +59,6 @@
     __builtin_amdgcn_sched_barrier(0);
   }
 #undef MN_LOAD
-}
-
-struct W1dRaw { float d[4]; };
-__device__ __forceinline__ W1dRaw w1d_raw(const float* p) { W1dRaw r; r.d[0] = p[0]; r.d[1] = p[1]; r.d[2] = p[2]; r.d[3] = p[3]; return r; }
-__device__ __forceinline__ void w1d_vr(const W1dRaw& r, float (&v)[4]) {
-  v[0] = r.d[0] - r.d[2]; v[1] = r.d[1] + r.d[2]; v[2] = r.d[2] - r.d[1]; v[3] = r.d[1] - r.d[3];
-}
-template <int NR, int SF = 2, int NCP = CK / 2, int CP0 = 0, int NKF = 3>
-__device__ __forceinline__ void chunk_w1d_s2(f32x16 (&acc)[4][2], const float* s_in, const float* s_w, int frel, int half, int l31) {
-  const float* wb = s_w + half * 32 + l31;
-  const float* ib0 = s_in + (half * NR + SF * frel) * TW + 2 * l31 + 3;
-  constexpr int NSTEP = NKF * NCP;
-  W1dRaw r0[2], r1[2];
-  float u[2][4];
-#define W1D_LOAD(ST, BUF)                                                                        \
-  {                                                                                              \
-    constexpr int kf_ = (ST) / NCP, cp_ = CP0 + (ST) % NCP;                                      \
-    const float* ib_ = ib0 + kf_ * TW + cp_ * 2 * NR * TW;                                       \
-    r0[BUF] = w1d_raw(ib_); r1[BUF] = w1d_raw(ib_ + 64);                                         \
-    _Pragma("unroll") for (int nu = 0; nu < 4; ++nu) u[BUF][nu] = wb[((nu * 3 + kf_) * CK + cp_ * 2) * 32]; \
-  }
-  W1D_LOAD(0, 0)
-#pragma unroll
-  for (int st = 0; st < NSTEP; ++st) {
-    const int cur = st & 1;
-    if (st + 1 < NSTEP) {
-      const int kf_ = (st + 1) / NCP, cp_ = CP0 + (st + 1) % NCP;
-      const float* ib_ = ib0 + kf_ * TW + cp_ * 2 * NR * TW;
-      r0[cur ^ 1] = w1d_raw(ib_); r1[cur ^ 1] = w1d_raw(ib_ + 64);
-#pragma unroll
-      for (int nu = 0; nu < 4; ++nu) u[cur ^ 1][nu] = wb[((nu * 3 + kf_) * CK + cp_ * 2) * 32];
-    }
-    __builtin_amdgcn_sched_barrier(0);
-    float v0[4], v1[4];
-    w1d_vr(r0[cur], v0);
-    w1d_vr(r1[cur], v1);
-#pragma unroll
-    for (int nu = 0; nu < 4; ++nu) {
-      acc[nu][0] = __builtin_amdgcn_mfma_f32_32x32x2f32(u[cur][nu], v0[nu], acc[nu][0], 0, 0, 0);
-      acc[nu][1] = __builtin_amdgcn_mfma_f32_32x32x2f32(u[cur][nu], v1[nu], acc[nu][1], 0, 0, 0);
-    }
-    __builtin_amdgcn_sched_barrier(0);
-  }
-#undef W1D_LOAD
-}
-__device__ __forceinline__ void chunk_w1d_tr2(f32x16 (&acc)[4][2], const float* s_in, const float* s_w, int pr, int q, int half, int l31) {
-  constexpr int NR = 3;
-  const float* wb = s_w + half * 32 + l31;
-  const float* ib = s_in + (half * NR + pr) * TW + 2 * l31 + 3 + 64 * q;
-  W1dRaw ra[2], rb[2];
-  float u0[2][4], u1[2][4], u2[2][4];
-#define W1D_LOAD(CP, BUF)                                                                        \
-  {                                                                                              \
-    ra[BUF] = w1d_raw(ib + (CP) * 2 * NR * TW); rb[BUF] = w1d_raw(ib + (CP) * 2 * NR * TW + TW); \
-    _Pragma("unroll") for (int nu = 0; nu < 4; ++nu) {                                           \
-      u0[BUF][nu] = wb[((nu * 3 + 0) * CK + (CP) * 2) * 32];                                     \
-      u1[BUF][nu] = wb[((nu * 3 + 1) * CK + (CP) * 2) * 32];                                     \
-      u2[BUF][nu] = wb[((nu * 3 + 2) * CK + (CP) * 2) * 32];                                     \
-    }                                                                                            \
-  }
-  W1D_LOAD(0, 0)
-#pragma unroll
-  for (int cp = 0; cp < CK / 2; ++cp) {
-    const int cur = cp & 1;
-    if (cp + 1 < CK / 2) W1D_LOAD(cp + 1, cur ^ 1)
-    __builtin_amdgcn_sched_barrier(0);
-    float va[4], vb[4];
-    w1d_vr(ra[cur], va);
-    w1d_vr(rb[cur], vb);
-#pragma unroll
-    for (int nu = 0; nu < 4; ++nu) {
-      acc[nu][0] = __builtin_amdgcn_mfma_f32_32x32x2f32(u0[cur][nu], va[nu], acc[nu][0], 0, 0, 0);
-      acc[nu][1] = __builtin_amdgcn_mfma_f32_32x32x2f32(u1[cur][nu], vb[nu], acc[nu][1], 0, 0, 0);
-      acc[nu][0] = __builtin_amdgcn_mfma_f32_32x32x2f32(u2[cur][nu], vb[nu], acc[nu][0], 0, 0, 0);
-    }
-    __builtin_amdgcn_sched_barrier(0);
-  }
-#undef W1D_LOAD
-}
-template <int Q0, int NQ, bool ACT = true>
-__device__ __forceinline__ void w1d_epilogue(const ConvArgs& a, f32x16 (&acc)[4][2], int n, int cg, int f, int tq, bool row_ok, int lane,
-                                             float* s_red, const float2* s_bc) {
-  const int half = lane >> 5, l31 = lane & 31;
-  const int T = a.T, Tp = a.Tp;
-  const int cbase = cg * 32;
-  const unsigned P4 = (unsigned)a.Fout * (unsigned)Tp * 4u;
-  const float* ob = a.out + (long long)n * a.out_bstride + (long long)a.out_c0 * a.Fout * Tp;
-  const __amdgpu_buffer_rsrc_t rs = make_rsrc_e(reinterpret_cast<unsigned long long>(ob), (unsigned)a.Cout * P4);
-  const bool all_t = row_ok && (tq + 64 * NQ <= T);
-  float2 bc[16];
-#pragma unroll
-  for (int r = 0; r < 16; ++r) bc[r] = s_bc[(r & 3) + 8 * (r >> 2) + 4 * half];
-  unsigned voff[NQ];
-  bool ok[NQ], ok2[NQ];
-#pragma unroll
-  for (int q = 0; q < NQ; ++q) {
-    const int te = tq + 64 * q + 2 * l31;
-    ok[q] = row_ok && te < T;
-    ok2[q] = ok[q] && te + 1 < T;
-    voff[q] = ok[q] ? (unsigned)(f * Tp + te) * 4u + (unsigned)(4 * half) * P4 : 0x80000000u;
-  }
-  float s1[16], s2[16];
-  auto body = [&](auto masked) {
-    constexpr bool MASKED = decltype(masked)::value;
-#pragma unroll
-    for (int r = 0; r < 16; ++r) {
-      const int kr = (r & 3) + 8 * (r >> 2);
-      const unsigned coff = (unsigned)(cbase + kr) * P4;
-      const float b = bc[r].x;
-      const f32x2_t cr = {bc[r].y, bc[r].y};
-      float a1 = 0.f, a2 = 0.f;
-#pragma unroll
-      for (int q = 0; q < NQ; ++q) {
-        const float m0 = acc[0][Q0 + q][r], m1 = acc[1][Q0 + q][r], m2 = acc[2][Q0 + q][r], m3 = acc[3][Q0 + q][r];
-        f32x2_t y = {(m0 + m1) + m2 + b, (m1 - m2) - m3 + b};
-        if (ACT) y = elu_fast2(y) - cr;
-        typedef unsigned int uu2 __attribute__((ext_vector_type(2)));
-        __builtin_amdgcn_raw_buffer_store_b64(__builtin_bit_cast(uu2, y), rs, voff[q] + coff, 0, 0);
-        if (!ACT) continue;
-        const float ze = (!MASKED || ok[q]) ? y.x : 0.f, zo = (!MASKED || ok2[q]) ? y.y : 0.f;
-        a1 += ze + zo;
-        a2 = fmaf(ze, ze, fmaf(zo, zo, a2));
-      }
-      s1[r] = a1;
-      s2[r] = a2;
-    }
-  };
-  if (all_t || !ACT) body(std::false_type{}); else body(std::true_type{});
-  if (!ACT) return;
-  const float x1 = reduce16_halfwave(s1, lane);
-  const float x2 = reduce16_halfwave(s2, lane);
-  if ((lane & 16) == 0) {
-    const int qq = lane & 15;
-    const int co_l = (qq & 3) + 8 * (qq >> 2) + 4 * half;
-    s_red[co_l * 2 + 0] = x1;
-    s_red[co_l * 2 + 1] = x2;
-  }
 }
 
 template <int NCO, int MODE, int OCTP = 0, bool HALFK = false, bool W1D = false>
@@ -508,6 +368,7 @@
   if ((e = set_lds_attr<1, 0, 4, true>()) != hipSuccess) return e;
 #endif
   if ((e = set_lds_attr<1, 0, 0, true>()) != hipSuccess) return e;
+  if ((e = conv_w1d_stream_init()) != hipSuccess) return e;
   return set_lds_attr<1, 0, 3, true>();
 }
 
@@ -558,6 +419,10 @@
   const dim3 gridw = conv_grid(a, n_samples, TT, FT, conv_xcd(n_samples));
   const size_t ldsw = conv_lds_bytes(a.NR, 32, a.Cin, 12);
   const bool w1d_half = ((a.Cin - 1) % CK) < CK / 2;
+  if (conv_w1d_stream_ok(sh, mode, false)) {
+    const hipError_t es = launch_conv_w1d_stream(a, mode, mode == 0 && w1d_half, s);
+    if (es != hipErrorNotSupported) return es;
+  }
   if (mode == 1) hipLaunchKernelGGL((conv3x3_mfma<1, 1, 0, false, true>), gridw, dim3(256), ldsw, s, a);
   else if (mode == 2) hipLaunchKernelGGL((conv3x3_mfma<1, 2, 0, false, true>), gridw, dim3(256), ldsw, s, a);
   else if (mode == 3) hipLaunchKernelGGL((conv3x3_mfma<1, 3, 0, false, true>), gridw, dim3(256), ldsw, s, a);
diff --git a/misonet_amd/csrc/conv_select.hpp b/misonet_amd/csrc/conv_select.hpp
--- a/misonet_amd/csrc/conv_select.hpp
+++ b/misonet_amd/csrc/conv_select.hpp
@@ -40,6 +40,7 @@
 }
 
 bool conv_w1d_ok(const ConvShape& s);
+bool conv_w1d_stream_ok(const ConvShape& s, int mode, bool one_row);
 bool conv_few_ok(const ConvShape& s);
 bool conv_wino_ok(const ConvShape& s);
 bool conv_x6_first_ok(const ConvShape& s);
diff --git a/misonet_amd/csrc/conv_w1d.hpp b/misonet_amd/csrc/conv_w1d.hpp
--- /dev/null
+++ b/misonet_amd/csrc/conv_w1d.hpp
@@ -0,0 +1,153 @@
+#pragma once
+#include "conv_epilogue.hpp"
+
+#include <type_traits>
+
+namespace mn {
+
+typedef float f32x16 __attribute__((ext_vector_type(16)));
+typedef float f32x4 __attribute__((ext_vector_type(4)));
+typedef unsigned int u32x4v __attribute__((ext_vector_type(4)));
+
+struct W1dRaw { float d[4]; };
+__device__ __forceinline__ W1dRaw w1d_raw(const float* p) { W1dRaw r; r.d[0] = p[0]; r.d[1] = p[1]; r.d[2] = p[2]; r.d[3] = p[3]; return r; }
+__device__ __forceinline__ void w1d_vr(const W1dRaw& r, float (&v)[4]) {
+  v[0] = r.d[0] - r.d[2]; v[1] = r.d[1] + r.d[2]; v[2] = r.d[2] - r.d[1]; v[3] = r.d[1] - r.d[3];
+}
+template <int NR, int SF = 2, int NCP = CK / 2, int CP0 = 0, int NKF = 3>
+__device__ __forceinline__ void chunk_w1d_s2(f32x16 (&acc)[4][2], const float* s_in, const float* s_w, int frel, int half, int l31) {
+  const float* wb = s_w + half * 32 + l31;
+  const float* ib0 = s_in + (half * NR + SF * frel) * TW + 2 * l31 + 3;
+  constexpr int NSTEP = NKF * NCP;
+  W1dRaw r0[2], r1[2];
+  float u[2][4];
+#define W1D_LOAD(ST, BUF)                                                                        \
+  {                                                                                              \
+    constexpr int kf_ = (ST) / NCP, cp_ = CP0 + (ST) % NCP;                                      \
+    const float* ib_ = ib0 + kf_ * TW + cp_ * 2 * NR * TW;                                       \
+    r0[BUF] = w1d_raw(ib_); r1[BUF] = w1d_raw(ib_ + 64);                                         \
+    _Pragma("unroll") for (int nu = 0; nu < 4; ++nu) u[BUF][nu] = wb[((nu * 3 + kf_) * CK + cp_ * 2) * 32]; \
+  }
+  W1D_LOAD(0, 0)
+#pragma unroll
+  for (int st = 0; st < NSTEP; ++st) {
+    const int cur = st & 1;
+    if (st + 1 < NSTEP) {
+      const int kf_ = (st + 1) / NCP, cp_ = CP0 + (st + 1) % NCP;
+      const float* ib_ = ib0 + kf_ * TW + cp_ * 2 * NR * TW;
+      r0[cur ^ 1] = w1d_raw(ib_); r1[cur ^ 1] = w1d_raw(ib_ + 64);
+#pragma unroll
+      for (int nu = 0; nu < 4; ++nu) u[cur ^ 1][nu] = wb[((nu * 3 + kf_) * CK + cp_ * 2) * 32];
+    }
+    __builtin_amdgcn_sched_barrier(0);
+    float v0[4], v1[4];
+    w1d_vr(r0[cur], v0);
+    w1d_vr(r1[cur], v1);
+#pragma unroll
+    for (int nu = 0; nu < 4; ++nu) {
+      acc[nu][0] = __builtin_amdgcn_mfma_f32_32x32x2f32(u[cur][nu], v0[nu], acc[nu][0], 0, 0, 0);
+      acc[nu][1] = __builtin_amdgcn_mfma_f32_32x32x2f32(u[cur][nu], v1[nu], acc[nu][1], 0, 0, 0);
+    }
+    __builtin_amdgcn_sched_barrier(0);
+  }
+#undef W1D_LOAD
+}
+__device__ __forceinline__ void chunk_w1d_tr2(f32x16 (&acc)[4][2], const float* s_in, const float* s_w, int pr, int q, int half, int l31) {
+  constexpr int NR = 3;
+  const float* wb = s_w + half * 32 + l31;
+  const float* ib = s_in + (half * NR + pr) * TW + 2 * l31 + 3 + 64 * q;
+  W1dRaw ra[2], rb[2];
+  float u0[2][4], u1[2][4], u2[2][4];
+#define W1D_LOAD(CP, BUF)                                                                        \
+  {                                                                                              \
+    ra[BUF] = w1d_raw(ib + (CP) * 2 * NR * TW); rb[BUF] = w1d_raw(ib + (CP) * 2 * NR * TW + TW); \
+    _Pragma("unroll") for (int nu = 0; nu < 4; ++nu) {                                           \
+      u0[BUF][nu] = wb[((nu * 3 + 0) * CK + (CP) * 2) * 32];                                     \
+      u1[BUF][nu] = wb[((nu * 3 + 1) * CK + (CP) * 2) * 32];                                     \
+      u2[BUF][nu] = wb[((nu * 3 + 2) * CK + (CP) * 2) * 32];                                     \
+    }                                                                                            \
+  }
+  W1D_LOAD(0, 0)
+#pragma unroll
+  for (int cp = 0; cp < CK / 2; ++cp) {
+    const int cur = cp & 1;
+    if (cp + 1 < CK / 2) W1D_LOAD(cp + 1, cur ^ 1)
+    __builtin_amdgcn_sched_barrier(0);
+    float va[4], vb[4];
+    w1d_vr(ra[cur], va);
+    w1d_vr(rb[cur], vb);
+#pragma unroll
+    for (int nu = 0; nu < 4; ++nu) {
+      acc[nu][0] = __builtin_amdgcn_mfma_f32_32x32x2f32(u0[cur][nu], va[nu], acc[nu][0], 0, 0, 0);
+      acc[nu][1] = __builtin_amdgcn_mfma_f32_32x32x2f32(u1[cur][nu], vb[nu], acc[nu][1], 0, 0, 0);
+      acc[nu][0] = __builtin_amdgcn_mfma_f32_32x32x2f32(u2[cur][nu], vb[nu], acc[nu][0], 0, 0, 0);
+    }
+    __builtin_amdgcn_sched_barrier(0);
+  }
+#undef W1D_LOAD
+}
+template <int Q0, int NQ, bool ACT = true, bool BCREG = true>
+__device__ __forceinline__ void w1d_epilogue(const ConvArgs& a, f32x16 (&acc)[4][2], int n, int cg, int f, int tq, bool row_ok, int lane,
+                                             float* s_red, const float2* s_bc) {
+  const int half = lane >> 5, l31 = lane & 31;
+  const int T = a.T, Tp = a.Tp;
+  const int cbase = cg * 32;
+  const unsigned P4 = (unsigned)a.Fout * (unsigned)Tp * 4u;
+  const float* ob = a.out + (long long)n * a.out_bstride + (long long)a.out_c0 * a.Fout * Tp;
+  const __amdgpu_buffer_rsrc_t rs = make_rsrc_e(reinterpret_cast<unsigned long long>(ob), (unsigned)a.Cout * P4);
+  const bool all_t = row_ok && (tq + 64 * NQ <= T);
+  float2 bc[BCREG ? 16 : 1];
+  if (BCREG) {
+#pragma unroll
+    for (int r = 0; r < 16; ++r) bc[BCREG ? r : 0] = s_bc[(r & 3) + 8 * (r >> 2) + 4 * half];
+  }
+  unsigned voff[NQ];
+  bool ok[NQ], ok2[NQ];
+#pragma unroll
+  for (int q = 0; q < NQ; ++q) {
+    const int te = tq + 64 * q + 2 * l31;
+    ok[q] = row_ok && te < T;
+    ok2[q] = ok[q] && te + 1 < T;
+    voff[q] = ok[q] ? (unsigned)(f * Tp + te) * 4u + (unsigned)(4 * half) * P4 : 0x80000000u;
+  }
+  float s1[16], s2[16];
+  auto body = [&](auto masked) {
+    constexpr bool MASKED = decltype(masked)::value;
+#pragma unroll
+    for (int r = 0; r < 16; ++r) {
+      const int kr = (r & 3) + 8 * (r >> 2);
+      const unsigned coff = (unsigned)(cbase + kr) * P4;
+      if (!BCREG) __builtin_amdgcn_sched_barrier(0);
+      const float2 bcr = BCREG ? bc[BCREG ? r : 0] : s_bc[kr + 4 * half];
+      const float b = bcr.x;
+      const f32x2_t cr = {bcr.y, bcr.y};
+      float a1 = 0.f, a2 = 0.f;
+#pragma unroll
+      for (int q = 0; q < NQ; ++q) {
+        const float m0 = acc[0][Q0 + q][r], m1 = acc[1][Q0 + q][r], m2 = acc[2][Q0 + q][r], m3 = acc[3][Q0 + q][r];
+        f32x2_t y = {(m0 + m1) + m2 + b, (m1 - m2) - m3 + b};
+        if (ACT) y = elu_fast2(y) - cr;
+        typedef unsigned int uu2 __attribute__((ext_vector_type(2)));
+        __builtin_amdgcn_raw_buffer_store_b64(__builtin_bit_cast(uu2, y), rs, voff[q] + coff, 0, 0);
+        if (!ACT) continue;
+        const float ze = (!MASKED || ok[q]) ? y.x : 0.f, zo = (!MASKED || ok2[q]) ? y.y : 0.f;
+        a1 += ze + zo;
+        a2 = fmaf(ze, ze, fmaf(zo, zo, a2));
+      }
+      s1[r] = a1;
+      s2[r] = a2;
+    }
+  };
+  if (all_t || !ACT) body(std::false_type{}); else body(std::true_type{});
+  if (!ACT) return;
+  const float x1 = reduce16_halfwave(s1, lane);
+  const float x2 = reduce16_halfwave(s2, lane);
+  if ((lane & 16) == 0) {
+    const int qq = lane & 15;
+    const int co_l = (qq & 3) + 8 * (qq >> 2) + 4 * half;
+    s_red[co_l * 2 + 0] = x1;
+    s_red[co_l * 2 + 1] = x2;
+  }
+}
+
+}
diff --git a/misonet_amd/csrc/conv_w1d_stream.hip b/misonet_amd/csrc/conv_w1d_stream.hip
--- /dev/null
+++ b/misonet_amd/csrc/conv_w1d_stream.hip
@@ -0,0 +1,307 @@
+#include "conv_select.hpp"
+#include "conv_w1d.hpp"
+#include "conv_w1d_stream.hpp"
+
+#include <atomic>
+
+namespace mn {
+
+__device__ __forceinline__ int opaque(int v) { asm volatile("" : "+v"(v)); return v; }
+
+constexpr int WS_RED = 8 * 32 * 2;
+
+template <int MODE, bool HALFK>
+__global__ __launch_bounds__(256, 2) void conv3x3_w1d_stream(const ConvArgs a, const unsigned ntiles) {
+  static_assert(MODE == 0 || (!HALFK && (MODE == 1 || MODE == 2)), "the first layers, the stride-2 convs, the stride-2 transposed convs");
+  constexpr int NR = MODE == 0 ? 6 : (MODE == 1 ? 9 : 3);
+  constexpr int SF = MODE == 1 ? 2 : 1;
+  constexpr bool TR2 = MODE == 2;
+  constexpr int NTAP = 12;
+  constexpr int NW4 = NTAP * CK * 32 / 4;
+  constexpr int NWI = NW4 / 256;
+  static_assert(NW4 % 256 == 0, "weight slab share per thread");
+  const int T = a.T, Tp = a.Tp, Fin = a.Fin, Cin = a.Cin;
+  const int nchunk = (Cin + CK - 1) / CK;
+  extern __shared__ __align__(16) float smem[];
+  float* s_in = smem;
+  float* s_w = s_in + CK * NR * TW;
+  float* s_red = s_w + NTAP * CK * 32;
+  float2* s_nrm = reinterpret_cast<float2*>(s_red + WS_RED);
+  float2* s_bc = s_nrm + nchunk * CK;
+
+  const int tid = threadIdx.x;
+  const int lane = tid & 63;
+  const int wave = __builtin_amdgcn_readfirstlane(tid >> 6);
+  const int half = lane >> 5, l31 = lane & 31;
+
+  const StreamRange rg = stream_range(ntiles, gridDim.x, blockIdx.x);
+  if (rg.count == 0) return;
+  int n, cg, f_tile, t_tile;
+  {
+    const StreamTile st = stream_tile(rg.first, a.ntx, a.nty, a.ncg);
+    n = st.n; cg = st.cg; f_tile = st.f_tile; t_tile = st.t_tile;
+  }
+
+  const int sq = tid & 31, sci = tid >> 5;
+  const int hr = tid >> 4, hci = (tid >> 1) & 7, hside = tid & 1;
+  const unsigned row_e = (unsigned)Tp;
+  const unsigned plane_e = (unsigned)Fin * row_e;
+
+  int t0, f0, fin0, tg;
+  bool hok, full_t;
+  unsigned hoff_b, toff_b;
+  __amdgpu_buffer_rsrc_t rs_in;
+  const f32x4* w_g;
+  f32x4 pin[NR];
+  float ph = 0.f;
+  f32x4 pw[NWI];
+
+#define TILE_SETUP()                                                                             \
+  {                                                                                              \
+    t0 = t_tile * TT;                                                                            \
+    f0 = f_tile * FT;                                                                            \
+    fin0 = TR2 ? (f0 >> 1) - 1 : SF * f0 - a.padf;                                               \
+    tg = t0 + 4 * sq;                                                                            \
+    const int htg_ = hside ? t0 + TT : t0 - 1;                                                   \
+    hok = (hr < NR) && htg_ >= 0 && htg_ < T && (fin0 + hr) >= 0 && (fin0 + hr) < Fin;           \
+    full_t = (t0 + TT <= T);                                                                     \
+    const unsigned long long pa_ = reinterpret_cast<unsigned long long>(                         \
+        a.in + (long long)n * a.in_bstride + (long long)a.in_c0 * Fin * Tp);                     \
+    const unsigned plo_ = __builtin_amdgcn_readfirstlane((unsigned)pa_);                         \
+    const unsigned phi_ = __builtin_amdgcn_readfirstlane((unsigned)(pa_ >> 32));                 \
+    rs_in = __builtin_amdgcn_make_buffer_rsrc(                                                   \
+        reinterpret_cast<void*>(((unsigned long long)phi_ << 32) | plo_), 0,                     \
+        __builtin_amdgcn_readfirstlane((int)((unsigned)Cin * plane_e * 4u)), 0x00020000);        \
+    w_g = reinterpret_cast<const f32x4*>(a.w1d + (long long)cg * nchunk * (NTAP * CK * 32));     \
+    const unsigned tg_e_ = (unsigned)(tg < Tp ? tg : Tp - 4);                                    \
+    {                                                                                            \
+      int fh_ = fin0 + (hr < NR ? hr : NR - 1);                                                  \
+      fh_ = fh_ < 0 ? 0 : (fh_ >= Fin ? Fin - 1 : fh_);                                          \
+      const int th_ = htg_ < 0 ? 0 : (htg_ >= Tp ? Tp - 1 : htg_);                               \
+      hoff_b = ((unsigned)fh_ * row_e + (unsigned)th_) * 4u;                                     \
+    }                                                                                            \
+    toff_b = tg_e_ * 4u;                                                                         \
+  }
+
+#define STAGE_ISSUE(KC)                                                                          \
+  {                                                                                              \
+    int c_ = (KC) * CK + sci;                                                                    \
+    c_ = c_ < Cin ? c_ : Cin - 1;                                                                \
+    const unsigned cb_ = (unsigned)c_ * plane_e * 4u;                                            \
+    _Pragma("unroll") for (int r = 0; r < NR; ++r) {                                             \
+      int fin_ = fin0 + r;                                                                       \
+      fin_ = fin_ < 0 ? 0 : (fin_ >= Fin ? Fin - 1 : fin_);                                      \
+      pin[r] = __builtin_bit_cast(f32x4, __builtin_amdgcn_raw_buffer_load_b128(                  \
+          rs_in, cb_ + toff_b, __builtin_amdgcn_readfirstlane((unsigned)fin_ * row_e * 4u), 0)); \
+    }                                                                                            \
+    int c2_ = (KC) * CK + hci;                                                                   \
+    c2_ = c2_ < Cin ? c2_ : Cin - 1;                                                             \
+    ph = __builtin_bit_cast(float, __builtin_amdgcn_raw_buffer_load_b32(                         \
+        rs_in, (unsigned)c2_ * plane_e * 4u + hoff_b, 0, 0));                                    \
+    const f32x4* wsrc_ = w_g + (unsigned)(KC) * (unsigned)NW4;                                   \
+    _Pragma("unroll") for (int i = 0; i < NWI; ++i) pw[i] = wsrc_[tid + 256 * i];                \
+  }
+
+#define STAGE_COMMIT(KC)                                                                         \
+  {                                                                                              \
+    const float2 m_ = s_nrm[(KC) * CK + sci];                                                    \
+    _Pragma("unroll") for (int r = 0; r < NR; ++r) {                                             \
+      const int fin_ = fin0 + r;                                                                 \
+      f32x4 v_ = {0.f, 0.f, 0.f, 0.f};                                                           \
+      if (fin_ >= 0 && fin_ < Fin) {                                                \
+        v_.x = fmaf(pin[r].x, m_.x, m_.y);                                                       \
+        v_.y = fmaf(pin[r].y, m_.x, m_.y);                                                       \
+        v_.z = fmaf(pin[r].z, m_.x, m_.y);                                                       \
+        v_.w = fmaf(pin[r].w, m_.x, m_.y);                                                       \
+        if (!full_t) {                                                                           \
+          v_.x = (tg + 0 < T) ? v_.x : 0.f;                                                      \
+          v_.y = (tg + 1 < T) ? v_.y : 0.f;                                                      \
+          v_.z = (tg + 2 < T) ? v_.z : 0.f;                                                      \
+          v_.w = (tg + 3 < T) ? v_.w : 0.f;                                                      \
+        }                                                                                        \
+      }                                                                                          \
+      *reinterpret_cast<f32x4*>(s_in + (sci * NR + r) * TW + 4 + 4 * sq) = v_;                   \
+    }                                                                                            \
+    if (hr < NR) {                                                                               \
+      const float2 m2_ = s_nrm[(KC) * CK + hci];                                                 \
+      s_in[(hci * NR + hr) * TW + (hside ? TT + 4 : 3)] = hok ? fmaf(ph, m2_.x, m2_.y) : 0.f;    \
+    }                                                                                            \
+    _Pragma("unroll") for (int i = 0; i < NWI; ++i) reinterpret_cast<f32x4*>(s_w)[tid + 256 * i] = pw[i]; \
+  }
+
+#define BUILD_TABLES()                                                                           \
+  {                                                                                              \
+    const int tid_ = opaque(tid);                                                                \
+    float bias_v_ = 0.f;                                                                         \
+    if (tid < 32) bias_v_ = __builtin_nontemporal_load(a.bias + cg * 32 + tid_);                 \
+    for (int c = tid_; c < nchunk * CK; c += 256) {                                               \
+      float mean = 0.f, rstd = (c < Cin) ? 1.f : 0.f;        \
+      if (c >= a.ident_c && c < Cin) {                                                           \
+        const dstat_t* st = a.in_stats + ((long long)n * a.in_sstride + a.in_c0 + c) * (2 * DS_NL); \
+        const double cnt = (double)Fin * (double)T;                                              \
+        const double m = dstat_read(st) / cnt;                                                   \
+        double var = dstat_read(st + DS_NL) / cnt - m * m;                                       \
+        var = var > 0.0 ? var : 0.0;                                                             \
+        mean = (float)m;                                                                         \
+        rstd = (float)(1.0 / sqrt(var + (double)IN_EPS));                                        \
+      }                                                                                          \
+      s_nrm[c] = make_float2(rstd, -mean * rstd);                                                \
+    }                                                                                            \
+    if (tid < 32) s_bc[tid] = make_float2(bias_v_, elu_fast(bias_v_));                           \
+  }
+
+  TILE_SETUP()
+  STAGE_ISSUE(0)
+  BUILD_TABLES()
+  __syncthreads();
+  STAGE_COMMIT(0)
+  __syncthreads();
+
+  for (unsigned it = 0; it < rg.count; ++it) {
+    const int e_n = n, e_cg = cg, e_f0 = f0, e_t0 = t0;
+    const int f = TR2 ? e_f0 + 2 * (wave >> 1) : e_f0 + wave;
+    const bool row_ok = f < a.Fout;
+
+    f32x16 wacc[4][2];
+#pragma unroll
+    for (int nu = 0; nu < 4; ++nu)
+#pragma unroll
+      for (int q = 0; q < 2; ++q)
+#pragma unroll
+        for (int r = 0; r < 16; ++r) wacc[nu][q][r] = 0.f;
+
+    for (int kc = 0; kc < nchunk; ++kc) {
+      const bool more = (kc + 1 < nchunk);
+      if (more) STAGE_ISSUE(kc + 1)
+      if (row_ok) {
+        if (TR2) chunk_w1d_tr2(wacc, s_in, s_w, wave >> 1, wave & 1, half, l31);
+        else if (HALFK) {
+          chunk_w1d_s2<NR, SF, CK / 4, 0>(wacc, s_in, s_w, f - e_f0, half, l31);
+          if (kc != nchunk - 1) chunk_w1d_s2<NR, SF, CK / 4, CK / 4>(wacc, s_in, s_w, f - e_f0, half, l31);
+        } else chunk_w1d_s2<NR, SF>(wacc, s_in, s_w, f - e_f0, half, l31);
+      }
+      __syncthreads();
+      if (more) {
+        STAGE_COMMIT(kc + 1)
+        __syncthreads();
+      }
+    }
+
+    const bool has_next = it + 1 < rg.count;
+    bool new_run = false;
+    if (has_next) {
+      if (++t_tile == a.ntx) {
+        t_tile = 0;
+        if (++f_tile == a.nty) {
+          f_tile = 0;
+          new_run = true;
+          if (++cg == a.ncg) { cg = 0; ++n; }
+        }
+      }
+      TILE_SETUP()
+      STAGE_ISSUE(0)
+    }
+
+    if (TR2) {
+      const int q = wave & 1, rt = 2 * (wave >> 1);
+      w1d_epilogue<0, 1, true, false>(a, wacc, e_n, e_cg, f, e_t0 + 64 * q, row_ok, lane, s_red + ((rt * 2 + q) * 32) * 2, s_bc);
+      w1d_epilogue<1, 1, true, false>(a, wacc, e_n, e_cg, f + 1, e_t0 + 64 * q, f + 1 < a.Fout, lane, s_red + (((rt + 1) * 2 + q) * 32) * 2, s_bc);
+    } else {
+      if (MODE == 0 && !a.act) w1d_epilogue<0, 2, false, false>(a, wacc, e_n, e_cg, f, e_t0, row_ok, lane, s_red + wave * (32 * 2), s_bc);
+      else w1d_epilogue<0, 2, true, false>(a, wacc, e_n, e_cg, f, e_t0, row_ok, lane, s_red + wave * (32 * 2), s_bc);
+    }
+
+    if (has_next) {
+      if (new_run) {
+        __syncthreads();
+        BUILD_TABLES()
+        __syncthreads();
+      }
+      STAGE_COMMIT(0)
+    }
+    __syncthreads();
+
+    if (a.act && tid < 64) {
+      const int tid_ = opaque(tid);
+      const int co_l = tid_ >> 1, which = tid_ & 1;
+      const int co = e_cg * 32 + co_l;
+      if (co < a.Cout) {
+        float tot = 0.f;
+        if (TR2) {
+          for (int sl = 0; sl < 8; ++sl)
+            if (e_f0 + (sl >> 1) < a.Fout) tot += s_red[(sl * 32 + co_l) * 2 + which];
+        } else {
+          for (int w = 0; w < FT; ++w)
+            if (e_f0 + w < a.Fout) tot += s_red[(w * 32 + co_l) * 2 + which];
+        }
+        dstat_add(a.out_stats + (((long long)e_n * a.out_sstride + a.out_c0 + co) * 2 + which) * DS_NL, (double)tot);
+      }
+    }
+  }
+}
+
+#undef TILE_SETUP
+#undef STAGE_ISSUE
+#undef STAGE_COMMIT
+#undef BUILD_TABLES
+
+static size_t stream_lds_bytes(int NR, int Cin) {
+  const int nchunk = (Cin + CK - 1) / CK;
+  return (size_t)(CK * NR * TW + 12 * CK * 32 + WS_RED) * sizeof(float) + (size_t)(nchunk * CK + 32) * sizeof(float2);
+}
+
+template <int MODE, bool HALFK>
+static hipError_t set_stream_attr() {
+  return hipFuncSetAttribute(reinterpret_cast<const void*>(&conv3x3_w1d_stream<MODE, HALFK>),
+                             hipFuncAttributeMaxDynamicSharedMemorySize, 96 * 1024);
+}
+
+hipError_t conv_w1d_stream_init() {
+  hipError_t e;
+  if ((e = set_stream_attr<0, false>()) != hipSuccess) return e;
+  if ((e = set_stream_attr<0, true>()) != hipSuccess) return e;
+  if ((e = set_stream_attr<1, false>()) != hipSuccess) return e;
+  return set_stream_attr<2, false>();
+}
+
+static std::atomic<int> g_stream_on{1};
+int conv_w1d_stream_switch(int on) {
+  if (on < 0) return g_stream_on.load(std::memory_order_relaxed);
+  return g_stream_on.exchange(on != 0, std::memory_order_relaxed);
+}
+
+constexpr int STREAM_PER_CU = 2;
+constexpr int STREAM_MAX_CIN = 2048;
+
+bool conv_w1d_stream_ok(const ConvShape& s, int mode, bool one_row) {
+  return !one_row && mode >= 0 && mode <= 2 && s.Cin >= 1 && s.Cin <= STREAM_MAX_CIN;
+}
+
+int conv_w1d_stream_schedule(int ntx, int nty, int ncg, int nsamp, int grid, int wg, int max_tiles, int* tiles) {
+  if (ntx <= 0 || nty <= 0 || ncg <= 0 || nsamp <= 0 || grid <= 0 || wg < 0 || wg >= grid || max_tiles < 0 || (max_tiles && !tiles)) return -1;
+  const long long nt = (long long)ntx * nty * ncg * nsamp;
+  if (nt > 0x7fffffffLL) return -1;
+  const StreamRange rg = stream_range((unsigned)nt, (unsigned)grid, (unsigned)wg);
+  for (unsigned i = 0; i < rg.count && (int)i < max_tiles; ++i) {
+    const StreamTile t = stream_tile(rg.first + i, ntx, nty, ncg);
+    tiles[4 * i + 0] = t.n; tiles[4 * i + 1] = t.cg; tiles[4 * i + 2] = t.f_tile; tiles[4 * i + 3] = t.t_tile;
+  }
+  return (int)rg.count;
+}
+
+hipError_t launch_conv_w1d_stream(const ConvArgs& a, int mode, bool halfk, hipStream_t s) {
+  if (!conv_w1d_stream_switch(-1)) return hipErrorNotSupported;
+  const long long nt = (long long)a.ntx * a.nty * a.ncg * a.nsamp;
+  const int cus = device_cus();
+  if (nt <= 0 || nt > 0x7fffffffLL || cus <= 0) return hipErrorNotSupported;
+  const unsigned ntiles = (unsigned)nt;
+  const dim3 grid(stream_grid(ntiles, cus, STREAM_PER_CU));
+  const size_t lds = stream_lds_bytes(a.NR, a.Cin);
+  if (mode == 1) hipLaunchKernelGGL((conv3x3_w1d_stream<1, false>), grid, dim3(256), lds, s, a, ntiles);
+  else if (mode == 2) hipLaunchKernelGGL((conv3x3_w1d_stream<2, false>), grid, dim3(256), lds, s, a, ntiles);
+  else if (halfk) hipLaunchKernelGGL((conv3x3_w1d_stream<0, true>), grid, dim3(256), lds, s, a, ntiles);
+  else hipLaunchKernelGGL((conv3x3_w1d_stream<0, false>), grid, dim3(256), lds, s, a, ntiles);
+  return hipGetLastError();
+}
+
+}
diff --git a/misonet_amd/csrc/conv_w1d_stream.hpp b/misonet_amd/csrc/conv_w1d_stream.hpp
--- /dev/null
+++ b/misonet_amd/csrc/conv_w1d_stream.hpp
@@ -0,0 +1,34 @@
+#pragma once
+#include <hip/hip_runtime.h>
+
+namespace mn {
+
+struct StreamRange { unsigned first, count; };
+struct StreamTile { int n, cg, f_tile, t_tile; };
+
+__host__ __device__ inline StreamRange stream_range(unsigned ntiles, unsigned G, unsigned w) {
+  const unsigned r = (G % 8u == 0u) ? (w & 7u) * (G >> 3) + (w >> 3) : w;
+  const unsigned q = ntiles / G, rem = ntiles - q * G;
+  StreamRange s;
+  s.first = r * q + (r < rem ? r : rem);
+  s.count = q + (r < rem ? 1u : 0u);
+  return s;
+}
+
+__host__ __device__ inline StreamTile stream_tile(unsigned idx, int ntx, int nty, int ncg) {
+  StreamTile t;
+  t.t_tile = (int)(idx % (unsigned)ntx); idx /= (unsigned)ntx;
+  t.f_tile = (int)(idx % (unsigned)nty); idx /= (unsigned)nty;
+  t.cg = (int)(idx % (unsigned)ncg);
+  t.n = (int)(idx / (unsigned)ncg);
+  return t;
+}
+
+inline unsigned stream_grid(unsigned ntiles, int cus, int per_cu) {
+  unsigned g = (unsigned)cus * (unsigned)per_cu;
+  g = g < ntiles ? g : ntiles;
+  if (g >= 8u) g &= ~7u;
+  return g;
+}
+
+}
diff --git a/misonet_amd/csrc/kernels.hpp b/misonet_amd/csrc/kernels.hpp
--- a/misonet_amd/csrc/kernels.hpp
+++ b/misonet_amd/csrc/kernels.hpp
@@ -94,6 +94,10 @@
 hipError_t launch_conv(const ConvArgs& a, int n_samples, hipStream_t s);
 hipError_t launch_conv_w1d(const ConvArgs& a, int n_samples, hipStream_t s);
 hipError_t conv_init();
+hipError_t launch_conv_w1d_stream(const ConvArgs& a, int mode, bool halfk, hipStream_t s);
+hipError_t conv_w1d_stream_init();
+int conv_w1d_stream_switch(int on);
+int conv_w1d_stream_schedule(int ntx, int nty, int ncg, int nsamp, int grid, int wg, int max_tiles, int* tiles);
 hipError_t launch_conv_wino(const ConvArgs& a, int n_samples, hipStream_t s);
 hipError_t conv_wino_init();
 hipError_t launch_conv_few(const ConvArgs& a, int n_samples, hipStream_t s);
diff --git a/misonet_amd/csrc/net.hip b/misonet_amd/csrc/net.hip
--- a/misonet_amd/csrc/net.hip
+++ b/misonet_amd/csrc/net.hip
@@ -598,7 +598,7 @@
   }
 }
 const char* misonet_last_error(void) { return g_err; }
-int misonet_version(void) { return 490; }
+int misonet_version(void) { return 500; }
 
 int misonet_net_create(const misonet_cfg* cfg, misonet_net** out) {
   if (!cfg || !out) return fail(MISONET_EINVAL, "null argument");
@@ -836,6 +836,13 @@
   return k;
 }
 
+int misonet_strided_stream(int on) { return conv_w1d_stream_switch(on); }
+
+int misonet_strided_schedule(int ntx, int nty, int ncg, int n_samples, int grid, int wg, int max_tiles, int* tiles) {
+  const int k = conv_w1d_stream_schedule(ntx, nty, ncg, n_samples, grid, wg, max_tiles, tiles);
+  return k < 0 ? fail(MISONET_EINVAL, "misonet_strided_schedule: bad geometry or workgroup index") : k;
+}
+
 int misonet_net_keep_activations(misonet_net* n, int keep) {
   if (!n) return fail(MISONET_EINVAL, "null argument");
   n->keep_taps = keep != 0;
```

Result: no change. 149.5 utt/s, median of 2 (+0.3%).
